# shoeffner/ann3depth

Measured on AMD Instinct MI355X. Metric: images/sec (640x480->55x74 MSDN train step), higher is better.
Workload: dtype f32

## Files before the change

### ann3depth_amd/_lib.py

```python
import collections
import ctypes
import os
from ctypes import c_char_p, c_float, c_int, c_int32, c_int64, c_size_t, c_uint8, c_uint32, c_void_p, POINTER

LIB_PATH = os.environ.get('A3D_LIB') or os.path.join(os.path.dirname(os.path.abspath(__file__)), 'liba3d.so')


class A3dError(RuntimeError):
    pass


class ConvDesc(ctypes.Structure):
    _fields_ = [(n, c_int32) for n in ('n', 'h', 'w', 'c', 'k', 'r', 's', 'stride', 'pad_t', 'pad_l', 'ho', 'wo',
                                       'ldx', 'ldy', 'precision', 'storage', 'hints')]


class SecondOutput(ctypes.Structure):
    _fields_ = [('ptr', c_void_p), ('ld', c_int32), ('step', c_int32), ('offset', c_int32), ('bf16', c_int32), ('cols', c_int32)]


class ExampleView(ctypes.Structure):
    _fields_ = [('image_height', c_int64), ('image_width', c_int64), ('image_channels', c_int64),
                ('depth_height', c_int64), ('depth_width', c_int64), ('depth_channels', c_int64),
                ('image', c_void_p), ('image_bytes', c_size_t), ('depth', c_void_p), ('depth_bytes', c_size_t)]
# ... 17 lines not shown
    'a3d_conv2d_bwd_filter_ws_bytes': (c_size_t, [_D]),
    'a3d_conv2d_bwd_filter': (c_int, [_D, _P, _P, _P, _P, _P, c_size_t, _P]),
    'a3d_conv2d_fwd_prepared_filter_bytes': (c_size_t, [_D]),
    'a3d_conv2d_fwd_prepare_filter': (c_int, [_D, _P, _P, c_size_t, _P]),
    'a3d_conv2d_bwd_filter_pooled_ws_bytes': (c_size_t, [_D]),
    'a3d_conv2d_bwd_filter_pooled': (c_int, [_D, _P, _P, c_int, _P, _P, c_int, c_int, _P, _P, _P, c_size_t, _P]),
    'a3d_conv2d_bwd_both_supported': (c_int, [_D]),
    'a3d_conv2d_bwd_both_ws_bytes': (c_size_t, [_D]),
    'a3d_conv2d_bwd_both': (c_int, [_D, _P, _P, _P, _P, _P, _P, c_int, c_int, c_int, _P, _P, c_size_t, _P]),
    'a3d_dense_fwd_ws_bytes': (c_size_t, [c_int, c_int, c_int]),
    'a3d_dense_fwd': (c_int, [c_int, c_int, c_int, _P, _P, _P, _P, c_int, _P, _P, c_size_t, _P]),
    'a3d_dense_bwd_data_ws_bytes': (c_size_t, [c_int, c_int, c_int]),
    'a3d_dense_bwd_data': (c_int, [c_int, c_int, c_int, _P, _P, _P, _P, c_int, c_float, _P, c_size_t, _P]),
    'a3d_dense_bwd_filter_ws_bytes': (c_size_t, [c_int, c_int, c_int]),
    'a3d_dense_bwd_filter': (c_int, [c_int, c_int, c_int, _P, _P, _P, _P, _P, c_size_t, _P]),
    'a3d_maxpool2x2_fwd': (c_int, [c_int, c_int, c_int, c_int, _P, _P, c_int, _P, _P]),
    'a3d_maxpool2x2_bwd': (c_int, [c_int, c_int, c_int, c_int, _P, _P, c_int, _P, c_int, _P]),
    'a3d_resize_bilinear_tf1': (c_int, [c_int, c_int, c_int, c_int, _P, c_int, c_int, _P, _P]),
    'a3d_resize_bilinear_tf1_pair': (c_int, [c_int, c_int, c_int, c_int, _P, c_int, c_int, _P, c_int, _P, c_int, c_int, _P, _P]),
    'a3d_resize_bilinear_tf1_ex': (c_int, [c_int, c_int, c_int, c_int, _P, c_int, c_int, c_int, _P, c_int, _P, c_int, c_int, c_int,
                                           _P, _P]),
    'a3d_warp_bilinear_pair': (c_int, [c_int, c_int, c_int, c_int, _P, c_int, c_int, c_int, _P, c_int, _P, c_int, c_int, c_int,
                                       _P, _P, _P]),
    'a3d_extract_patches': (c_int, [c_int, c_int, c_int, c_int, _P, c_int, c_int, _P, _P]),
    'a3d_silog_loss_fwd': (c_int, [c_int, c_int, _P, _P, _P, _P, _P]),
    'a3d_silog_loss_bwd': (c_int, [c_int, c_int, _P, _P, _P, _P, _P]),
    'a3d_dropout_keep_mask': (c_int, [c_size_t, ctypes.c_uint64, ctypes.c_uint64, c_float, _P, _P]),
    'a3d_adam_apply_tf1': (c_int, [c_size_t, _P, _P, _P, _P, c_float, c_float, c_float, c_float, c_float, c_float,
                                   c_float, _P]),
    'a3d_adam_apply_tf1_flag': (c_int, [c_size_t, _P, _P, _P, _P, c_float, c_float, c_float, c_float, c_float, c_float,
                                        c_float, _P, _P]),
    'a3d_dense_fwd_ex': (c_int, [c_int, c_int, c_int, _P, _P, _P, _P, c_int, _P, c_int, c_int, _P, c_size_t, _P]),
    'a3d_dense_bwd_data_ex': (c_int, [c_int, c_int, c_int, _P, _P, _P, _P, c_int, c_float, c_int, c_int, _P, c_size_t, _P]),
    'a3d_dense_fwd_ex2': (c_int, [c_int, c_int, c_int, _P, _P, _P, _P, c_int, c_int, c_int, _P, c_int, c_int, POINTER(SecondOutput), _P,
                                  c_size_t, _P]),
    'a3d_dense_bwd_data_ex2': (c_int, [c_int, c_int, c_int, _P, _P, _P, _P, c_int, c_float, c_int, c_int, POINTER(SecondOutput), _P,
                                       c_size_t, _P]),
    'a3d_conv2d_fwd_ex2': (c_int, [_D, _P, _P, _P, _P, c_int, POINTER(SecondOutput), _P, c_size_t, _P]),
    'a3d_silog_loss_bwd_ex': (c_int, [c_int, c_int, _P, _P, _P, _P, _P, c_int, _P]),
    'a3d_depth_metrics_ws_bytes': (c_size_t, [c_int, c_int, c_int]),
    'a3d_depth_metrics': (c_int, [c_int, c_int, c_int, _P, c_int, c_int, _P, c_int, c_float, c_float, c_float, c_float, _P, _P,
                                  c_size_t, _P]),
    'a3d_cast_bf16': (c_int, [c_size_t, _P, _P, c_int, _P]),
    'a3d_cast_rows': (c_int, [c_size_t, c_int, _P, c_int, c_int, _P, c_int, c_int, _P]),
    'a3d_pad_channels_bf16': (c_int, [c_size_t, c_int, _P, c_int, _P, _P]),
    'a3d_stream_create': (c_int, [c_int, ctypes.POINTER(ctypes.c_void_p)]),
    'a3d_stream_destroy': (c_int, [_P]),
    'a3d_maxpool2x2_fwd_bf16': (c_int, [c_int, c_int, c_int, c_int, _P, c_int, _P, c_int, _P, _P]),
    'a3d_maxpool2x2_bwd_bf16': (c_int, [c_int, c_int, c_int, c_int, _P, c_int, _P, c_int, _P, c_int, _P]),
    'a3d_copy_channel_bf16': (c_int, [c_size_t, _P, c_int, c_int, _P, c_int, c_int, _P]),
    'a3d_maxpool2x2_bwd_idx_bf16': (c_int, [c_int, c_int, c_int, c_int, _P, _P, c_int, _P, c_int, _P, c_int, _P]),
    'a3d_maxpool2x2_bwd_idx_bf16s': (c_int, [c_int, c_int, c_int, c_int, _P, _P, c_int, _P, c_int, _P, c_int, _P]),
    'a3d_dense_bwd_filter_adam_tf1': (c_int, [c_int, c_int, c_int, _P, _P, _P, _P, _P, _P, _P, _P, c_float, c_float, c_float,
                                              c_float, c_float, c_float, _P]),
    'a3d_dense_bwd_filter_adam_tf1_ex': (c_int, [c_int, c_int, c_int, _P, _P, _P, _P, _P, _P, _P, _P, c_float, c_float, c_float,
                                                 c_float, c_float, c_float, c_int, _P]),
    'a3d_superpixel_mean': (c_int, [c_int, c_int, c_int, c_int, _P, c_int, _P, _P]),
    'a3d_superpixel_hist': (c_int, [c_int, c_int, c_int, _P, c_int, _P, _P]),
    'a3d_pair_similarity': (c_int, [c_int, c_int, c_int, _P, c_int, _P, _P, _P, c_int, _P, _P, c_float, _P, _P, _P]),
    'a3d_crf_loss': (c_int, [c_int, c_int, _P, _P, _P, _P, _P, c_int, c_float, _P, _P, _P, _P]),
    'a3d_crf_map': (c_int, [c_int, c_int, _P, _P, _P, _P, c_int, _P, _P, _P]),
    'a3d_sgd_apply': (c_int, [c_size_t, _P, _P, c_float, _P]),
    'a3d_conv2d_pool_fwd': (c_int, [_D, _P, _P, _P, _P, c_int, _P, c_int, _P, c_size_t, _P]),
    'a3d_maxpool2x2_bwd_idx': (c_int, [c_int, c_int, c_int, c_int, _P, _P, c_int, _P, c_int, _P, c_int, _P]),
    'a3d_copy_channel': (c_int, [c_size_t, _P, c_int, c_int, _P, c_int, c_int, _P]),
    'a3d_comm_standin': (c_int, [_P, c_size_t, _P, c_size_t, c_int, c_float, _P]),
    'a3d_timing_enable': (c_int, [c_int]),
    'a3d_timing_collect': (c_int, [POINTER(TimingRecord), c_int]),
    'a3d_timing_select': (c_int, [POINTER(TimingRecord)]),
    'a3d_crc32c': (c_uint32, [_P, c_size_t]),
    'a3d_masked_crc32c': (c_uint32, [_P, c_size_t]),
    'a3d_tfrecord_next': (c_int, [_P, c_size_t, c_int, POINTER(c_size_t), POINTER(c_size_t), POINTER(c_size_t)]),
    'a3d_example_parse': (c_int, [_P, c_size_t, POINTER(ExampleView)]),
    'a3d_decode_raw_plus_half': (c_int, [_P, c_size_t, _P]),
    'a3d_record_decode': (c_int, [_P, c_size_t, c_int, _P, c_size_t, _P, c_size_t, POINTER(ExampleView)]),
    'a3d_record_decode_u8': (c_int, [_P, c_size_t, c_int, _P, _P, c_size_t, _P, _P, c_size_t, POINTER(ExampleView),
                                     POINTER(c_int)]),
    'a3d_records_decode': (c_int, [POINTER(c_void_p), POINTER(c_size_t), c_int, c_int, POINTER(c_int64), _P, _P, _P, _P,
                                   POINTER(c_int32), c_int, POINTER(c_int32)]),
    'a3d_h2d_gather': (c_int, [_P, _P, POINTER(c_int32), c_int, c_int, c_size_t, _P]),
    'a3d_sizeof_conv_desc': (c_size_t, []),
    'a3d_example_write': (c_int64, [_P, c_int, c_int, c_int, _P, c_int, c_int, c_int, _P, c_size_t]),
}

EXT_SIGNATURES = {
    'a3dx_resize_bilinear_tf1_valid': (c_int, [c_int, c_int, c_int, c_int, _P, c_int, c_int, c_int, _P, c_int, _P, c_int, c_int,
                                               c_int, _P, c_float, c_float, _P]),
    'a3dx_warp_bilinear_pair_valid': (c_int, [c_int, c_int, c_int, c_int, _P, c_int, c_int, c_int, _P, c_int, _P, c_int, c_int,
                                              c_int, _P, _P, c_float, c_float, _P]),
    'a3dx_silog_masked_loss_fwd': (c_int, [c_int, c_int, _P, _P, _P, _P, _P]),
    'a3dx_silog_masked_loss_bwd_ex': (c_int, [c_int, c_int, _P, _P, _P, _P, _P, c_int, _P]),
}

PAIR_SIGNATURES = {
    'a3dp_crf_loss_grad': (c_int, [c_int, c_int, _P, _P, _P, _P, _P, c_int, c_float, _P, _P, _P, _P, _P]),
    'a3dp_pair_dense_bwd': (c_int, [c_int, c_int, c_int, _P, _P, _P, _P, _P]),
    'a3dp_sgd_apply_floor': (c_int, [c_size_t, _P, _P, c_float, c_float, _P]),
}

TEXTURE_SIGNATURES = {
    'a3dt_superpixel_lbp_hist': (c_int, [c_int, c_int, c_int, _P, c_int, _P, _P]),
    'a3dt_pair_similarity3': (c_int, [c_int, c_int, c_int, _P, c_int, _P, _P, _P, _P, c_int, _P, _P, c_float, _P, _P, _P]),
}

GRADLOSS_SIGNATURES = {
    'a3dg_silog_grad_loss_fwd': (c_int, [c_int, c_int, c_int, _P, _P, c_int, c_float, _P, _P, _P]),
    'a3dg_silog_grad_loss_bwd_ex': (c_int, [c_int, c_int, c_int, _P, _P, c_int, c_float, _P, _P, _P, c_int, _P]),
}

BERHU_SIGNATURES = {
    'a3dh_berhu_loss_fwd': (c_int, [c_int, c_int, _P, _P, c_int, c_float, _P, _P, _P]),
    'a3dh_berhu_loss_bwd_ex': (c_int, [c_int, c_int, _P, _P, c_int, c_float, _P, _P, _P, c_int, _P]),
}

ALIGN_SIGNATURES = {
    'a3da_depth_align_ws_bytes': (c_size_t, [c_int, c_int, c_int, c_int]),
    'a3da_depth_align': (c_int, [c_int, c_int, c_int, _P, c_int, c_int, _P, c_int, c_float, c_float, c_int, _P, _P, _P, _P,
                                 c_size_t, _P]),
    'a3da_depth_metrics_aligned': (c_int, [c_int, c_int, c_int, _P, c_int, c_int, _P, c_int, c_float, c_float, c_float, c_float,
                                           _P, _P, _P, c_size_t, _P]),
    'a3da_affine_apply': (c_int, [c_int, c_int, _P, _P, _P, _P]),
}

SSI_SIGNATURES = {
    'a3di_ssi_loss_fwd': (c_int, [c_int, c_int, _P, _P, c_int, _P, _P, _P]),
    'a3di_ssi_loss_bwd_ex': (c_int, [c_int, c_int, _P, _P, c_int, _P, _P, _P, c_int, _P]),
}

CRF_VALID_SIGNATURES = {
    'a3dv_superpixel_mean_valid': (c_int, [c_int, c_int, c_int, _P, c_int, c_int, _P, _P, _P]),
    'a3dv_crf_loss_observed': (c_int, [c_int, c_int, _P, _P, _P, _P, _P, c_int, _P, _P, _P, _P, _P, _P, _P]),
}

FCSP_SIGNATURES = {
    'a3df_superpixel_pool_fwd': (c_int, [c_int, c_int, c_int, c_int, _P, c_int, c_int, c_int, c_int, _P, _P, _P, c_int, _P]),
    'a3df_superpixel_pool_bwd': (c_int, [c_int, c_int, c_int, c_int, _P, c_int, c_int, c_int, c_int, _P, _P, _P, c_int, _P]),
}

CRF_BAND_SIGNATURES = {
    'a3db_crf_band_nll': (c_int, [c_int, c_int, c_int, _P, _P, _P, _P, _P, c_int, _P, _P, _P, _P, _P, _P, _P]),
    'a3db_crf_band_map': (c_int, [c_int, c_int, c_int, _P, _P, _P, _P, c_int, _P, _P, _P]),
}

WINO_SIGNATURES = {
    'a3dw_conv2d_bwd_data_prepared_filter_bytes': (c_size_t, [_D]),
    'a3dw_conv2d_bwd_data_prepare_filter': (c_int, [_D, _P, _P, c_size_t, _P]),
}

WINO_GRAD_SIGNATURES = {
    'a3dwg_conv2d_bwd_filter_ws_bytes': (c_size_t, [_D]),
    'a3dwg_conv2d_bwd_filter': (c_int, [_D, _P, _P, _P, _P, _P, c_size_t, _P]),
}

class WinoBwdPool(ctypes.Structure):
    _fields_ = [('argmax', c_void_p), ('y', c_void_p), ('ldy', c_int), ('h2', c_int), ('w2', c_int)]


WINO_BWD_SIGNATURES = {
    'a3dwb_sizeof_pool': (c_size_t, []),
    'a3dwb_conv2d_bwd_ws_bytes': (c_size_t, [_D, c_int, c_int]),
    'a3dwb_conv2d_bwd': (c_int, [_D, _P, _P, _P, _P, _P, _P, _P, ctypes.POINTER(WinoBwdPool), _P, c_size_t, _P]),
}

UPSAMPLE_SIGNATURES = {
    'a3du_joint_bilateral_upsample': (c_int, [c_int, c_int, c_int, _P, c_int, c_int, _P, c_int, _P, _P, _P, _P, c_int, c_float,
                                              c_float, _P, _P]),
}

POSTERIOR_SIGNATURES = {
    'a3dc_crf_band_posterior': (c_int, [c_int, c_int, c_int, _P, _P, _P, _P, _P, c_int, _P, _P, _P, _P, _P]),
}

SLIC_SIGNATURES = {
    'a3ds_label_mean': (c_int, [c_int, c_int, c_int, c_int, _P, c_int, _P, _P, _P, _P]),
    'a3ds_label_hist': (c_int, [c_int, c_int, c_int, _P, c_int, _P, _P, _P]),
    'a3ds_slic_update': (c_int, [c_int, c_int, c_int, _P, c_int, _P, _P, _P, _P]),
    'a3ds_slic_assign': (c_int, [c_int, c_int, c_int, _P, c_int, _P, c_float, _P, _P]),
    'a3ds_slic_segment': (c_int, [c_int, c_int, c_int, _P, c_int, c_int, c_float, _P, _P, _P, _P]),
    'a3ds_pair_similarity': (c_int, [c_int, c_int, _P, _P, _P, _P, _P, c_int, _P, _P, c_float, _P, _P, _P]),
    'a3ds_label_pool_fwd': (c_int, [c_int, c_int, c_int, c_int, _P, c_int, c_int, c_int, c_int, _P, _P, _P, _P, _P, c_int, _P]),
    'a3ds_label_pool_bwd': (c_int, [c_int, c_int, c_int, c_int, _P, c_int, c_int, c_int, c_int, _P, _P, _P, _P, _P, c_int, _P]),
}

Surface = collections.namedtuple('Surface', 'prefix header signatures')
SURFACES = (
    Surface('a3d_', 'a3d.h', SIGNATURES),
    Surface('a3dx_', 'a3d_valid.h', EXT_SIGNATURES),
    Surface('a3dp_', 'a3d_pairwise.h', PAIR_SIGNATURES),
    Surface('a3dt_', 'a3d_texture.h', TEXTURE_SIGNATURES),
    Surface('a3dg_', 'a3d_gradloss.h', GRADLOSS_SIGNATURES),
    Surface('a3dv_', 'a3d_crf_valid.h', CRF_VALID_SIGNATURES),
    Surface('a3df_', 'a3d_fcsp.h', FCSP_SIGNATURES),
    Surface('a3db_', 'a3d_crf_band.h', CRF_BAND_SIGNATURES),
    Surface('a3dw_', 'a3d_wino.h', WINO_SIGNATURES),
    Surface('a3du_', 'a3d_upsample.h', UPSAMPLE_SIGNATURES),
    Surface('a3dc_', 'a3d_posterior.h', POSTERIOR_SIGNATURES),
    Surface('a3dwg_', 'a3d_wino_grad.h', WINO_GRAD_SIGNATURES),
    Surface('a3ds_', 'a3d_slic.h', SLIC_SIGNATURES),
    Surface('a3dwb_', 'a3d_wino_bwd.h', WINO_BWD_SIGNATURES),
    Surface('a3dh_', 'a3d_berhu.h', BERHU_SIGNATURES),
    Surface('a3da_', 'a3d_align.h', ALIGN_SIGNATURES),
    Surface('a3di_', 'a3d_ssi.h', SSI_SIGNATURES),
)

_lib = None


def load():
    global _lib
    if _lib is not None:
        return _lib
    if not os.path.exists(LIB_PATH):
        raise A3dError(f'{LIB_PATH} not found: build it with `python -c "import __graft_entry__ as g; g.build()"` '
                       f'or `make -C ann3depth_amd/csrc` (there is no fallback path)')
    import torch
    lib = ctypes.CDLL(LIB_PATH)
    for name, (res, args) in ((n, sig) for surface in SURFACES for n, sig in surface.signatures.items()):
        try:
            fn = getattr(lib, name)
        except AttributeError as e:
            raise A3dError(f'liba3d.so lacks symbol {name}: stale build?') from e
        fn.restype = res
        fn.argtypes = args
    if lib.a3d_sizeof_conv_desc() != ctypes.sizeof(ConvDesc):
        raise A3dError(f'liba3d.so reads a {lib.a3d_sizeof_conv_desc()}-byte a3d_conv_desc, this binding passes '
                       f'{ctypes.sizeof(ConvDesc)} bytes: stale build?')
    if lib.a3dwb_sizeof_pool() != ctypes.sizeof(WinoBwdPool):
        raise A3dError(f'liba3d.so reads a {lib.a3dwb_sizeof_pool()}-byte a3dwb_pool, this binding passes '
                       f'{ctypes.sizeof(WinoBwdPool)} bytes: stale build?')
    _lib = lib
    return lib


def last_error():
    buf = ctypes.create_string_buffer(512)
    load().a3d_last_error(buf, 512)
    return buf.value.decode(errors='replace')


def check(rc, what):
    if rc != 0:
        raise A3dError(f'{what} failed ({rc}): {last_error()}')
```

### ann3depth_amd/csrc/a3d_internal.h

```cpp
#pragma once
#include <hip/hip_runtime.h>
#include <stddef.h>
#include <stdint.h>

#include <algorithm>

#include "../../include/a3d.h"
#include "igemm_plan.h"

namespace a3d {

int set_error(int code, const char* fmt, ...);

#define A3D_CHECK_ARG(cond, ...)                                 \
  do {                                                           \
    if (!(cond)) return ::a3d::set_error(A3D_EINVAL, __VA_ARGS__); \
  } while (0)

inline void clear_stale_error() { (void)hipGetLastError(); }

inline int check_launch(const char* what) {
  hipError_t e = hipGetLastError();
  if (e != hipSuccess) return set_error(A3D_ELAUNCH, "%s: %s", what, hipGetErrorString(e));
  return A3D_OK;
}

inline unsigned grid_for(size_t total, int per_block = 256, unsigned cap = 8192) {
  size_t g = (total + per_block - 1) / per_block;
  return (unsigned)std::min<size_t>(std::max<size_t>(g, 1), cap);
}

__host__ __device__ inline bool aligned16(const void* p) { return (reinterpret_cast<uintptr_t>(p) & 15) == 0; }

struct IgemmParams;
int launch_igemm(int mode, const GemmPlan& plan, int avec, int bvec, IgemmParams& p, void* ws, hipStream_t st);
int take_second_output(IgemmParams& p, const a3d_second_output* o);

struct TimingSlot {
  hipEvent_t start, stop;
  a3d_timing_record rec;
};
bool timing_wanted(const a3d_timing_record& r);
int timing_begin(TimingSlot& slot, hipStream_t st);
void timing_end(TimingSlot& slot, hipStream_t st);
a3d_timing_record timing_record(int mode, int prec, int bm, int bn, int waves_m, int nwaves, int bk, int avec, int bvec, int lds_dma,
                                int m, int n, int k);
template <typename Launch>
int timed_launch(const a3d_timing_record& rec, hipStream_t st, Launch&& launch) {
  if (!timing_wanted(rec)) return launch();
  TimingSlot slot{};
  slot.rec = rec;
  int rc = timing_begin(slot, st);
  if (rc != A3D_OK) return rc;
  rc = launch();
  timing_end(slot, st);
  return rc;
}

bool dense_dw_applicable(int m, int k, int n);
bool dense_stream_applicable(int m, int k, int n);
size_t dense_stream_ws_bytes(int m, int k, int n);
int dense_fwd_stream(int m, int k, int n, const float* x, const float* w, const float* bias, float* y, int act,
                     const uint8_t* keep, float keep_scale, void* ws, size_t ws_bytes, hipStream_t st);
struct ReduceParams;
int launch_splitk_reduce(const ReduceParams& r, hipStream_t st);
int dense_dw_launch(int m, int k, int n, const float* x, const float* dz, float* dw, float* db, hipStream_t st);

size_t colsum_bf16_ws_bytes(int n);
bool colsum_bf16_ok(int n);
int colsum_bf16(const void* dz, int rows, int n, int ld, float* out, void* ws, int* nparts, hipStream_t st);

bool stencil1_applicable(const a3d_conv_desc* d);
size_t stencil1_bwdf_ws_bytes(const a3d_conv_desc* d);
int stencil1_fwd(const a3d_conv_desc* d, const float* x, const float* w, const float* bias, float* y, int act,
                 hipStream_t st);
int stencil1_bwd_filter(const a3d_conv_desc* d, const float* x, const float* dz, float* dw, float* db, void* ws,
                        hipStream_t st);
bool stencil1_bwd_both_applicable(const a3d_conv_desc* d);
size_t stencil1_bwd_both_ws_bytes(const a3d_conv_desc* d);
int stencil1_bwd_both(const a3d_conv_desc* d, const float* x, const float* dz, const float* w, float* dw, float* db,
                      void* dx, int lddx, int dx_bf16, int relu_mask, unsigned* state, void* ws, hipStream_t st);

bool fewch_bwdf_applicable(const a3d_conv_desc* d, bool pooled);
size_t fewch_bwdf_ws_bytes(const a3d_conv_desc* d, bool pooled);
bool fewch_extents_ok(const a3d_conv_desc* d, bool pooled, int ldz, int esz, int ld_arg);
int fewch_bwd_filter(const a3d_conv_desc* d, const float* x, int src, const void* dz, int ldz, const void* pooled_act,
                     const uint8_t* argmax, int ld_arg, float* dw, float* db, void* ws, hipStream_t st);

int fewch_reduce_launch(const float* slabs, int splits, int Mp, int NP, int M, int N, float* dw, float* db, hipStream_t st);
bool fewch16_bwdf_applicable(const a3d_conv_desc* d, bool pooled);
size_t fewch16_bwdf_ws_bytes(const a3d_conv_desc* d, bool pooled);
int fewch16_bwd_filter(const a3d_conv_desc* d, const float* x, bool pooled, const void* dz, int ldz, const void* pooled_act,
                       const uint8_t* argmax, int ld_arg, float* dw, float* db, void* ws, hipStream_t st);

bool conv3_applicable(const a3d_conv_desc* d, unsigned x_off);
size_t conv3_ws_bytes(const a3d_conv_desc* d);
int conv3_pack(const a3d_conv_desc* d, const float* w, float* wp, hipStream_t st);
int conv3_fwd(const a3d_conv_desc* d, const float* x, const float* w, const float* bias, float* y, int act, int pool,
              int ld_out, uint8_t* argmax, void* ws, size_t ws_bytes, hipStream_t st, bool prepared = false);

bool conv3b_applicable(const a3d_conv_desc* d);
size_t conv3b_filter_bytes(const a3d_conv_desc* d);
int conv3b_pack(const a3d_conv_desc* d, const float* w, void* wp, hipStream_t st);
int conv3b_fwd(const a3d_conv_desc* d, const void* x, const float* w, const float* bias, void* y, int act, int pool, int ld_out,
               uint8_t* argmax, void* ws, size_t ws_bytes, hipStream_t st, bool prepared);

struct WinoGeom {
  int oh, ow, th, tw;
  size_t T;
  int K, N, Kp, Np;
  size_t v_bytes, m_bytes, u_bytes;
};
WinoGeom wino_geom(const a3d_conv_desc* d, bool bwd);
bool wino_applicable(const a3d_conv_desc* d);
int wino_filter(const a3d_conv_desc* d, bool bwd, const float* w, float* U, hipStream_t st);
int wino_input(const a3d_conv_desc* d, bool bwd, const float* src, float* V, hipStream_t st);
int wino_output(const a3d_conv_desc* d, bool bwd, const float* M, float* out, const float* bias, const float* mask, int act,
                hipStream_t st);
a3d_timing_record wino_record(int mode, const WinoGeom& g);
int wino_gemm(IgemmParams& p, const WinoGeom& g, hipStream_t st);

struct WinoGradGeom {
  size_t T;
  int Cp, Kp;
  int splits;
  size_t v_bytes, z_bytes;
  size_t slab_bytes, bias_bytes;
};
int wino_grad_splits(int C, int K, size_t T);
WinoGradGeom wino_grad_geom(const a3d_conv_desc* d);
bool wino_grad_applicable(const a3d_conv_desc* d);
int wino_dz(const a3d_conv_desc* d, const float* dz, float* Z, hipStream_t st);
int wino_dw(const a3d_conv_desc* d, const WinoGradGeom& g, const float* slabs, const float* bparts, float* dw, float* db, hipStream_t st);
a3d_timing_record wino_grad_record(const a3d_conv_desc* d, const WinoGradGeom& g);
int wino_grad_gemm(IgemmParams& p, const WinoGradGeom& g, hipStream_t st);

struct WinoBwdPool {
  const uint8_t* argmax;
  const float* y;
  int ldy, h2, w2;
};
int wino_bwd_transforms(const a3d_conv_desc* d, const float* x, const float* dz, float* Vx, float* Vdz, float* Z, hipStream_t st);
int wino_bwd_gemm(IgemmParams& pf, const WinoGradGeom& gg, IgemmParams& pd, const WinoGeom& g, hipStream_t st);
int wino_bwd_finish(const a3d_conv_desc* d, const WinoGradGeom& gg, const float* slabs, const float* bparts, float* dw, float* db,
                    const float* M, float* dx, const float* mask, const WinoBwdPool* pool, hipStream_t st);

}
```

### ann3depth_amd/csrc/igemm.h

```cpp
#pragma once
#include <hip/hip_runtime.h>
#include <stdint.h>

#include <type_traits>

#include "igemm_plan.h"

namespace a3d {

#ifdef A3D_STAMPS
#define A3D_STAMP(var)                                                                         \
  do {                                                                                         \
    __builtin_amdgcn_sched_barrier(0);                                                         \
    unsigned long long t_;                                                                     \
    asm volatile("s_memtime %0\n\ts_waitcnt lgkmcnt(0)" : "=s"(t_)::"memory");                 \
    __builtin_amdgcn_sched_barrier(0);                                                         \
    var = t_;                                                                                  \
  } while (0)
#define A3D_RTSTAMP(var)                                                                       \
  do {                                                                                         \
    __builtin_amdgcn_sched_barrier(0);                                                         \
    unsigned long long t_;                                                                     \
    asm volatile("s_memrealtime %0\n\ts_waitcnt lgkmcnt(0)" : "=s"(t_)::"memory");             \
    __builtin_amdgcn_sched_barrier(0);                                                         \
// ... 918 lines not shown
    const int kt = kt_begin + it;
    const bool more = it + 1 < nkt;
    A3D_STAMP(s0);
    if (AHEAD) issue();
    else prepare(uni_c, std::true_type{}, kt + 1, (it + 1) % 3, more);
    __builtin_amdgcn_sched_barrier(0);
    A3D_STAMP(s1);
    if (AHEAD) prepare(uni_c, std::false_type{}, kt + 2, (it + 2) % 3, it + 2 < nkt);
    if (MODE == MODE_BWD_F) {
      if (tid < Cfg::PIX) pixtab[((it + 2) % 3) * Cfg::PIX + tid] = row_entry((kt + 2) * BK + tid, image_of((kt + 2) * BK));
    }
    const float* Ac = As + cur * Cfg::A_ELEMS;
    const float* Bc = Bs + cur * Cfg::B_ELEMS;
    if (MODE == MODE_BWD_F && do_bias) {
#pragma unroll 8
      for (int k = 0; k < BK; ++k) bsum += Bc[k * Cfg::B_LD + (tid ^ (Cfg::B_SWZ ? 32 * ((k >> 2) & 1) : 0))];
    }
    constexpr bool PIPE = (MODE != MODE_FWD) && NWAVES == 8 && BN == 128;
    if constexpr (PIPE) {
      f32x4 af[2][TM], bf[2][TN];
      auto read_frags = [&](int u, int buf) {
        const int kk = 8 * u + 4 * lh;
#pragma unroll
        for (int a = 0; a < TM; ++a) {
          const int row = (wm * Cfg::WM + a * 32 + li) ^ (Cfg::A_SWZ ? 32 * lh : 0);
          if (MODE == MODE_BWD_F) {
#pragma unroll
            for (int j = 0; j < 4; ++j) af[buf][a][j] = Ac[(kk + j) * Cfg::A_LD + row];
          } else {
            af[buf][a] = *reinterpret_cast<const f32x4*>(Ac + row * Cfg::A_LD + kk);
          }
        }
#pragma unroll
        for (int b = 0; b < TN; ++b) {
          const int col = (wn * Cfg::WN + b * 32 + li) ^ (Cfg::B_SWZ ? 32 * lh : 0);
          if (MODE == MODE_BWD_D) {
            bf[buf][b] = *reinterpret_cast<const f32x4*>(Bc + col * Cfg::B_LD + kk);
          } else {
#pragma unroll
            for (int j = 0; j < 4; ++j) bf[buf][b][j] = Bc[(kk + j) * Cfg::B_LD + col];
          }
        }
      };
      read_frags(0, 0);
#pragma unroll
      for (int u = 0; u < BK / 8; ++u) {
        constexpr int LAST = BK / 8 - 1;
        if (u < LAST) read_frags(u + 1, (u + 1) & 1);
        if (u == LAST) {
          A3D_STAMP(s2);
          if (more) store_tiles(cur ^ 1);
          A3D_STAMP(s3);
        }
#pragma unroll
        for (int j = 0; j < 4; ++j)
#pragma unroll
          for (int a = 0; a < TM; ++a)
#pragma unroll
            for (int b = 0; b < TN; ++b)
              acc[a][b] = __builtin_amdgcn_mfma_f32_32x32x2f32(af[u & 1][a][j], bf[u & 1][b][j], acc[a][b], 0, 0, 0);
        if (u < LAST) {
          constexpr int NREADS = (MODE == MODE_BWD_F ? 4 * (TM + TN) : TM + TN);
          constexpr int NMFMA = 4 * TM * TN;
          constexpr int PER = (NREADS + NMFMA - 1) / NMFMA;
#pragma unroll
          for (int i = 0; i < NMFMA; ++i) {
            __builtin_amdgcn_sched_group_barrier(0x008, 1, 0);
            __builtin_amdgcn_sched_group_barrier(0x100, PER, 0);
          }
        }
      }
    } else {
#pragma unroll
    for (int u = 0; u < BK / 8; ++u) {
      f32x4 af[TM], bf[TN];
      const int kk = 8 * u + 4 * lh;
#pragma unroll
      for (int a = 0; a < TM; ++a) {
        const int row = (wm * Cfg::WM + a * 32 + li) ^ (Cfg::A_SWZ ? 32 * lh : 0);
        if (MODE == MODE_BWD_F) {
#pragma unroll
          for (int j = 0; j < 4; ++j) af[a][j] = Ac[(kk + j) * Cfg::A_LD + row];
        } else {
          af[a] = *reinterpret_cast<const f32x4*>(Ac + row * Cfg::A_LD + kk);
        }
      }
#pragma unroll
      for (int b = 0; b < TN; ++b) {
        const int col = (wn * Cfg::WN + b * 32 + li) ^ (Cfg::B_SWZ ? 32 * lh : 0);
        if (MODE == MODE_BWD_D) {
          bf[b] = *reinterpret_cast<const f32x4*>(Bc + col * Cfg::B_LD + kk);
        } else {
#pragma unroll
          for (int j = 0; j < 4; ++j) bf[b][j] = Bc[(kk + j) * Cfg::B_LD + col];
        }
      }
      if (u == BK / 8 - 1) {
        A3D_STAMP(s2);
        if (more) store_tiles(cur ^ 1);
        A3D_STAMP(s3);
      }
#pragma unroll
      for (int j = 0; j < 4; ++j)
#pragma unroll
        for (int a = 0; a < TM; ++a)
#pragma unroll
          for (int b = 0; b < TN; ++b)
            acc[a][b] = __builtin_amdgcn_mfma_f32_32x32x2f32(af[a][j], bf[b][j], acc[a][b], 0, 0, 0);
    }
    }
    A3D_STAMP(s4);
    __syncthreads();
    A3D_STAMP(s5);
#ifdef A3D_STAMPS
    d01 += s1 - s0; d12 += s2 - s1; d23 += s3 - s2; d34 += s4 - s3; d45 += s5 - s4;
#endif
  };
  for (int it = 0; it < nkt; it += 2) {
    tile_body(it, std::integral_constant<int, 0>{});
    if (it + 1 < nkt) tile_body(it + 1, std::integral_constant<int, 1>{});
  }
  };
  if constexpr (MODE == MODE_BWD_F) {
    k_loop(std::false_type{});
  } else {
    if (p.uni) k_loop(std::true_type{});
    else k_loop(std::false_type{});
  }
#ifdef A3D_STAMPS
  A3D_STAMP(tend);
  A3D_RTSTAMP(rtend);
  if (p.stamps && lane == 0) {
    unsigned long long* o = p.stamps + ((size_t)bid_in * NWAVES + wave) * 16;
    o[0] = d01; o[1] = d12; o[2] = d23; o[3] = d34; o[4] = d45; o[5] = tend - tbeg; o[6] = (unsigned long long)nkt; o[7] = tp1 - t_entry; o[15] = tp2 - tp1;
    o[8] = tbeg - t_entry; o[9] = t_entry; o[10] = tend; o[12] = rtend - rtbeg; o[13] = rtbeg; o[14] = rtend;
  }
#define A3D_STAMP_EXIT()                                                                                   \
  do {                                                                                                     \
    unsigned long long t_exit_;                                                                            \
    A3D_STAMP(t_exit_);                                                                                    \
    if (p.stamps && lane == 0) p.stamps[((size_t)bid_in * NWAVES + wave) * 16 + 11] = t_exit_;              \
  } while (0)
#else
#define A3D_STAMP_EXIT() do { } while (0)
#endif

  igemm_epilogue<MODE, BM, BN, TM, TN, Cfg::WM, Cfg::WN>(p, acc, split, bid, seg, kt_begin, kt_end, nk_total, do_bias, bsum, tid, wave, lane,
                                                          m0, n0, wm, wn);
  }
  A3D_STAMP_EXIT();
}

template <int MODE, int BM, int BN, int WAVES_M, int NWAVES>
__global__ __launch_bounds__(256) void igemm_fixup_kernel(const IgemmParams p, const uint32_t nblk) {
  constexpr int WAVES_N = NWAVES / WAVES_M, WM = BM / WAVES_M, WN = BN / WAVES_N, TM = WM / 32, TN = WN / 32;
  constexpr int UNITS = NWAVES * TM * TN * 4;
  constexpr int MAXC = 1024;
  __shared__ uint32_t slots[MAXC];
  __shared__ uint32_t nslots;
  const int lane = threadIdx.x & 63;
  const int unit = (int)blockIdx.y * 4 + (int)(threadIdx.x >> 6);
  const uint32_t tile = blockIdx.x;
  const uint32_t nk = p.div_nk.d, tiles = (uint32_t)(p.tiles_m * p.tiles_n);
  if (threadIdx.x == 0) {
    uint32_t n = 0;
    const uint32_t total = tiles * nk, t0 = tile * nk, t1 = t0 + nk - 1;
    uint32_t jf = (uint32_t)(((unsigned long long)t0 * nblk) / total), jl = (uint32_t)(((unsigned long long)t1 * nblk) / total);
    while (jf + 1 < nblk && sk_first(jf + 1, nblk, total) <= t0) ++jf;
    while (jl + 1 < nblk && sk_first(jl + 1, nblk, total) <= t1) ++jl;
    for (uint32_t b = jf; b <= jl; ++b) {
      const uint32_t f = sk_first(b, nblk, total);
      if (f == sk_first(b + 1, nblk, total)) continue;
      if (n < MAXC) slots[n] = 2 * b + (f / nk == tile ? 0u : 1u);
      ++n;
    }
    nslots = n < MAXC ? n : MAXC;
  }
  __syncthreads();
  const uint32_t n = nslots;
  if (n <= 1) return;
  const int tile_m = (int)tile / p.tiles_n, tile_n = (int)tile - tile_m * p.tiles_n;
  if (unit < UNITS) {
    const size_t uoff = ((size_t)unit * 64 + lane) * 4;
    f32x4 s = {0.f, 0.f, 0.f, 0.f};
    auto slab_of = [&](uint32_t i) -> f32x4 {
      return *reinterpret_cast<const f32x4*>(p.sk_ws + (size_t)slots[i] * (size_t)(BM * BN) + uoff);
    };
    uint32_t i = 0;
    for (; i + 8 <= n; i += 8) {
      f32x4 v[8];
#pragma unroll
      for (int u = 0; u < 8; ++u) v[u] = slab_of(i + u);
#pragma unroll
      for (int u = 0; u < 8; ++u) s += v[u];
    }
    if (i + 4 <= n) {
      const f32x4 v0 = slab_of(i), v1 = slab_of(i + 1), v2 = slab_of(i + 2), v3 = slab_of(i + 3);
      s += v0; s += v1; s += v2; s += v3;
      i += 4;
    }
    for (; i < n; ++i) s += slab_of(i);
    const int q = unit & 3, ab = unit >> 2, bb = ab % TN, a = (ab / TN) % TM, wave = ab / (TN * TM);
    const int wm = wave / WAVES_N, wn = wave % WAVES_N, li = lane & 31, lh = lane >> 5;
    store_quad<MODE>(p, s, tile_m * BM + wm * WM + a * 32 + 8 * q + 4 * lh, tile_n * BN + wn * WN + bb * 32 + li, p.C,
                     p.ldc, false);
  }
  if (MODE == MODE_BWD_F && p.dbias != nullptr && tile_m == 0 && blockIdx.y == 0 && (int)threadIdx.x < BN) {
    static_assert(BN <= 256, "bias sums by the first 256 threads");
    float bsum = 0.f;
    for (uint32_t i = 0; i < n; ++i) bsum += p.sk_bias[(size_t)slots[i] * BN + threadIdx.x];
    if (tile_n * BN + (int)threadIdx.x < p.N) p.dbias[tile_n * BN + threadIdx.x] = bsum;
  }
}

template <int MODE, int BM, int BN, int WAVES_M, int NWAVES, int BKT, int AVEC, int BVEC>
__global__ __launch_bounds__(64 * NWAVES, (BKT == 16 ? 3 : 2) * NWAVES / 4) void igemm_kernel(const IgemmParams p) {
  igemm_body<MODE, BM, BN, WAVES_M, NWAVES, BKT, AVEC, BVEC>(p, gridDim.x, blockIdx.x);
}

struct IgemmMulti {
  IgemmParams p[4];
};
template <int MODE, int BM, int BN, int WAVES_M, int NWAVES, int BKT, int AVEC, int BVEC>
__global__ __launch_bounds__(64 * NWAVES, (BKT == 16 ? 3 : 2) * NWAVES / 4) void igemm_multi_kernel(const IgemmMulti ps) {
  const IgemmParams& p = ps.p[blockIdx.y];
  const uint32_t nwg = (uint32_t)(p.tiles_m * p.tiles_n * p.splitk);
  if (blockIdx.x >= nwg) return;
  igemm_body<MODE, BM, BN, WAVES_M, NWAVES, BKT, AVEC, BVEC>(p, nwg, blockIdx.x);
}

struct ReduceParams {
  const float* ws; float* C; const float* bias; const float* mask; const uint8_t* keep; float mask_scale;
  int M, N, ldc, splitk, act, mode, mask_act; size_t slab;
  int sub_step, sub_ph, sub_pw, outW, outHW; FastDiv div_phw, div_pw;
  int vec4;
  int c16;
  const float* dbias_ws; float* dbias_out;
  int dbias_splits;
  unsigned dbias_block0;
  void* C2; int ld2, step2, off2, c2_16, cols2;
  int c_cols;
  int row_rl, row_rlp;
};
__global__ __launch_bounds__(256) void splitk_reduce_kernel(const ReduceParams p);

}
```

### ann3depth_amd/csrc/igemm_host.hip

```cpp
#include <algorithm>
#include <cmath>

#include "../../include/a3d_wino.h"
#include "../../include/a3d_wino_grad.h"
#include "../../include/a3d_wino_bwd.h"
#include "a3d_internal.h"
#include "igemm.h"
#include "igemm_cfgs.h"

namespace a3d {

int launch_igemm_multi_bwd_d(int avec, int bvec, IgemmMulti& ps, unsigned grid_x, unsigned count, hipStream_t st);
int launch_igemm_bf16_multi_bwd_d(int bn, IgemmMulti& ps, unsigned grid_x, unsigned count, hipStream_t st);


struct RunForm {
  int vec;
  int rl, rlp;
  int kp;
  int np;
  size_t bytes;
};
static bool run_form_ok(const a3d_conv_desc* d, unsigned x_off, RunForm* rf, bool bwd_filter = false) {
  if (d->pad_t || d->pad_l || d->ldx != d->c || d->c % 4 == 0 || d->c > 4) return false;
  const int step = d->stride * d->c, row = d->w * d->c;
  int vec = 0;
  bool anywhere = false;
  if (step % 4 == 0 && row % 4 == 0 && x_off == 0) vec = 4;
  else if (step % 2 == 0 && row % 2 == 0 && (x_off & 7) == 0) vec = 2;
  else if (bwd_filter && d->precision == A3D_PREC_F32 && !d->storage && (x_off & 3) == 0) {
    vec = 2;
    anywhere = true;
  }
  if (vec == 4 && d->precision == A3D_PREC_F32) {
    const int rl = d->s * d->c;
    const int kp4 = d->r * ((rl + 3) / 4 * 4), kp2 = d->r * ((rl + 1) / 2 * 2);
    if ((kp2 + 127) / 128 < (kp4 + 127) / 128) vec = 2;
  }
  if (!vec) return false;
  rf->vec = vec;
  rf->rl = d->s * d->c;
  rf->rlp = (rf->rl + vec - 1) / vec * vec;
  rf->kp = d->r * rf->rlp;
  rf->np = (d->k + 3) / 4 * 4;
  rf->bytes = ((size_t)rf->kp * rf->np * 4 + 255) / 256 * 256;
  if (anywhere) return (d->wo - 1) * step + rf->rl <= row && (d->ho - 1) * d->stride + d->r <= d->h;
  return (d->wo - 1) * step + rf->rlp <= row;
}

__global__ __launch_bounds__(256) void pad_filter_kernel(const float* w, float* wp, int r, int rl, int rlp, int n, int np) {
  const int total = r * rlp * np;
  for (int i = blockIdx.x * 256 + threadIdx.x; i < total; i += gridDim.x * 256) {
    const int col = i % np, row = i / np;
    const int q = row % rlp, rr = row / rlp;
    wp[i] = (q < rl && col < n) ? w[(size_t)(rr * rl + q) * n + col] : 0.f;
  }
}
__global__ __launch_bounds__(256) void unpad_filter_kernel(const float* wp, float* w, int r, int rl, int rlp, int n) {
  const int total = r * rl * n;
  for (int i = blockIdx.x * 256 + threadIdx.x; i < total; i += gridDim.x * 256) {
    const int col = i % n, row = i / n;
    const int q = row % rl, rr = row / rl;
    w[i] = wp[(size_t)(rr * rlp + q) * n + col];
  }
}

struct Operands {
  bool known = false;
  unsigned x = 0, w = 0, y = 0;
  unsigned aux = 0;
  int act = A3D_ACT_NONE, pool = 0, ld_out = 0;
  bool argmax = false, prepared = false;
  bool db = true;
};
static const Operands kOnGrid{};
static Operands launch_operands(const void* x, const void* w, const void* y, const void* aux) {
  auto off16 = [](const void* p) { return (unsigned)(reinterpret_cast<uintptr_t>(p) & 15); };
  Operands o;
  o.known = true;
  o.x = off16(x); o.w = off16(w); o.y = off16(y); o.aux = off16(aux);
  return o;
}

enum GemmForm { kAsStored, kLdsDma, kRunForm, kBf16Image };
struct Route {
  bool ok = false;
  RunForm rf{};
  GemmProblem g{};
  GemmPlan plan{};
  size_t repack = 0;
  size_t bytes = 0;
};
static size_t upto(size_t need, const Route& r) { return r.ok ? std::max(need, r.bytes) : need; }
static void fit_workspace(Route& r, const Operands& o, size_t ws_bytes, size_t per_split = 0) {
  if (r.bytes <= ws_bytes || !(o.x | o.w | o.y | o.aux) || r.repack > ws_bytes) return;
  r.plan = plan_within(r.g, r.plan, ws_bytes - r.repack, per_split);
  r.bytes = r.repack + r.plan.ws_bytes + (r.plan.splitk > 1 ? (size_t)r.plan.splitk * per_split : 0);
}
#define A3D_CHECK_WS(ws, who) A3D_CHECK_ARG(aligned16(ws), who ": ws must be 16-byte aligned")

static const int kAll16 = A3D_STORE_X_BF16 | A3D_STORE_W_BF16 | A3D_STORE_Y_BF16;
static bool stored16(const a3d_conv_desc* d, int bits) { return (d->storage & bits) == bits; }
static bool ring_ok(const a3d_conv_desc* d, const Operands& o, int both, unsigned out_off, int taps) {
  if (d->precision != A3D_PREC_BF16 || !stored16(d, both) || d->c % 8 || d->k % 8) return false;
  return !o.known || (d->ldx % 8 == 0 && d->ldy % 8 == 0 && taps <= 128 && !out_off);
}

static int ilog2_exact(int v) {
  for (int l = 0; l < 8; ++l)
    if ((1 << l) == v) return l;
  return -1;
}

static int check_desc(const a3d_conv_desc* d) {
  A3D_CHECK_ARG(d != nullptr, "conv: null descriptor");
  A3D_CHECK_ARG(d->n > 0 && d->h > 0 && d->w > 0 && d->c > 0 && d->k > 0 && d->r > 0 && d->s > 0, "conv: bad dims");
  A3D_CHECK_ARG(ilog2_exact(d->stride) >= 0 && d->stride <= 4, "conv: stride %d unsupported (1, 2 or 4)", d->stride);
  A3D_CHECK_ARG(d->pad_t >= 0 && d->pad_l >= 0 && d->pad_t < d->r && d->pad_l < d->s, "conv: bad padding");
  A3D_CHECK_ARG(d->ho > 0 && d->wo > 0, "conv: bad output size");
  A3D_CHECK_ARG((d->ho - 1) * d->stride - d->pad_t < d->h && (d->wo - 1) * d->stride - d->pad_l < d->w,
                "conv: output size inconsistent with input");
  A3D_CHECK_ARG(d->ldx >= d->c && d->ldy >= d->k, "conv: pixel strides smaller than channel counts");
  A3D_CHECK_ARG(d->precision >= A3D_PREC_F32 && d->precision <= A3D_PREC_F32_WINOGRAD, "conv: unknown precision %d", d->precision);
  const double lim = 2147483647.0;
  A3D_CHECK_ARG((double)d->n * d->h * d->w * d->ldx < lim && (double)d->n * d->ho * d->wo * d->ldy < lim &&
                    (double)d->r * d->s * d->c * d->k < lim,
                "conv: tensor too large for 31-bit indexing");
  auto tile_span_ok = [&](double rows_per_image, double image_elems) {
    const double images = std::min((double)d->n, std::floor(255.0 / rows_per_image) + 2.0);
    return images * image_elems * 4.0 < lim;
  };
  A3D_CHECK_ARG(tile_span_ok((double)d->ho * d->wo, (double)d->h * d->w * d->ldx) &&
                    tile_span_ok(std::max(1.0, std::floor((double)d->h / d->stride) * std::floor((double)d->w / d->stride)),
                                 (double)d->ho * d->wo * d->ldy),
                "conv: single images too large for 31-bit byte offsets inside a tile");
  return A3D_OK;
}

#define A3D_AS_F32(d)                                          \
  a3d_conv_desc d##_f32;                                       \
  if ((d) && (d)->precision == A3D_PREC_F32_WINOGRAD) {        \
    d##_f32 = *(d);                                            \
    d##_f32.precision = A3D_PREC_F32;                          \
    (d) = &d##_f32;                                            \
  }

static GemmProblem fwd_problem(const a3d_conv_desc* d) {
  GemmProblem g;
  g.mode = MODE_FWD;
  g.M = d->n * d->ho * d->wo; g.N = d->k; g.K = d->r * d->s * d->c;
  g.avec = (d->c % 4 == 0 && d->ldx % 4 == 0) ? 4 : 1;
  g.bvec = (d->k % 4 == 0) ? 4 : 1;
  return g;
}
static GemmProblem bwd_d_problem(const a3d_conv_desc* d) {
  GemmProblem g;
  g.mode = MODE_BWD_D;
  g.M = d->n * d->h * d->w; g.N = d->c; g.K = d->r * d->s * d->k;
// ... 648 lines not shown
  fill_common(p, r.g);
  rc = apply_storage(p, d->precision, d->storage & A3D_STORE_X_BF16, d->storage & A3D_STORE_Y_BF16, false, d->c, d->ldx, -1, d->ldy,
                     x, dz, dw, "x", "dz", "dw");
  if (rc != A3D_OK) return rc;
  A3D_CHECK_ARG(!d->storage || plan.prec == A3D_PREC_BF16, "conv2d_bwd_filter: bf16 storage needs vectorisable operands");
  if (r.bytes > ws_bytes) return set_error(A3D_EWORKSPACE, "conv2d_bwd_filter: need %zu workspace bytes", r.bytes);
  hipStream_t st = static_cast<hipStream_t>(stream);
  if (plan.ring && db) {
    float* parts = reinterpret_cast<float*>(static_cast<char*>(ws) + plan.ws_bytes);
    int nparts = 0;
    rc = colsum_bf16(dz, r.g.K, d->k, d->ldy, plan.splitk > 1 ? nullptr : db, parts, &nparts, st);
    if (rc != A3D_OK) return rc;
    if (plan.splitk > 1) { p.dbias_parts = parts; p.dbias_parts_out = db; p.dbias_parts_n = nparts; }
    db = nullptr;
  }
  p.A = x; p.B = dz; p.C = out; p.dbias = db;
  p.npix = r.g.K; p.nrsc = r.g.M;
  fill_gather(p, d, d->ldx, run ? 1 : d->s, run ? rf.rlp : d->c);
  p.ldb = d->ldy; p.ldc = d->k;
  fill_staging(p, MODE_BWD_F, (unsigned long long)d->n * d->h * d->w * d->ldx, (unsigned long long)d->n * d->ho * d->wo * d->ldy, d->r,
               run ? 1 : d->s);
  if (run) { p.unpad_dst = dw; p.unpad_rl = rf.rl; p.unpad_rlp = rf.rlp; }
  rc = launch_igemm(MODE_BWD_F, plan, r.g.avec, r.g.bvec, p, static_cast<char*>(ws) + r.repack, st);
  if (rc != A3D_OK || !run || p.unpad_done) return rc;
  clear_stale_error();
  hipLaunchKernelGGL(unpad_filter_kernel, dim3((d->r * rf.rl * d->k + 255) / 256), dim3(256), 0, st, out, dw, d->r,
                     rf.rl, rf.rlp, d->k);
  return check_launch("unpad_filter");
}

static bool wino_grad_takes(const a3d_conv_desc* d) { return check_desc(d) == A3D_OK && wino_grad_applicable(d); }

static IgemmParams wino_grad_product(const WinoGradGeom& g, const float* V, const float* Z, float* slabs, float* bparts) {
  a3d_conv_desc e{};
  e.n = (int)g.T; e.h = e.w = e.ho = e.wo = 1; e.c = g.Cp; e.k = g.Kp; e.r = e.s = 1; e.stride = 1; e.ldx = g.Cp; e.ldy = g.Kp;
  GemmProblem gp = bwd_f_problem(&e);
  IgemmParams p;
  fill_common(p, gp);
  p.A = V; p.B = Z; p.C = slabs; p.dbias = bparts;
  p.npix = gp.K; p.nrsc = gp.M;
  fill_gather(p, &e, g.Cp, 1, g.Cp);
  p.ldb = g.Kp; p.ldc = g.Kp;
  fill_staging(p, MODE_BWD_F, (unsigned long long)g.T * g.Cp, (unsigned long long)g.T * g.Kp, 1, 1);
  return p;
}

size_t a3dwg_conv2d_bwd_filter_ws_bytes(const a3d_conv_desc* d) {
  if (!wino_grad_takes(d)) return a3d_conv2d_bwd_filter_ws_bytes(d);
  const WinoGradGeom g = wino_grad_geom(d);
  return g.v_bytes + g.z_bytes + g.slab_bytes + g.bias_bytes;
}

int a3dwg_conv2d_bwd_filter(const a3d_conv_desc* d, const float* x, const float* dz, float* dw, float* db, void* ws,
                            size_t ws_bytes, void* stream) {
  if (!wino_grad_takes(d)) return a3d_conv2d_bwd_filter(d, x, dz, dw, db, ws, ws_bytes, stream);
  A3D_CHECK_ARG(x && dz && dw, "conv2d_bwd_filter (Winograd): null tensor");
  A3D_CHECK_WS(ws, "conv2d_bwd_filter (Winograd)");
  const WinoGradGeom g = wino_grad_geom(d);
  const size_t need = g.v_bytes + g.z_bytes + g.slab_bytes + g.bias_bytes;
  if (!ws || need > ws_bytes) return set_error(A3D_EWORKSPACE, "conv2d_bwd_filter (Winograd): need %zu workspace bytes", need);
  hipStream_t st = static_cast<hipStream_t>(stream);
  char* base = static_cast<char*>(ws);
  float* V = reinterpret_cast<float*>(base);
  float* Z = reinterpret_cast<float*>(base + g.v_bytes);
  float* slabs = reinterpret_cast<float*>(base + g.v_bytes + g.z_bytes);
  float* bparts = reinterpret_cast<float*>(base + g.v_bytes + g.z_bytes + g.slab_bytes);
  int rc = wino_input(d, false, x, V, st);
  if (rc != A3D_OK) return rc;
  rc = wino_dz(d, dz, Z, st);
  if (rc != A3D_OK) return rc;
  IgemmParams p = wino_grad_product(g, V, Z, slabs, db ? bparts : nullptr);
  rc = timed_launch(wino_grad_record(d, g), st, [&] { return wino_grad_gemm(p, g, st); });
  if (rc != A3D_OK) return rc;
  return wino_dw(d, g, slabs, bparts, dw, db, st);
}

static bool wino_bwd_takes(const a3d_conv_desc* d) {
  if (!wino_grad_takes(d)) return false;
  const WinoGeom gx = wino_geom(d, false), gd = wino_geom(d, true);
  return gx.th <= gd.th && gx.tw <= gd.tw;
}
static a3d_conv_desc as_winograd(const a3d_conv_desc* d) {
  a3d_conv_desc e = *d;
  e.precision = A3D_PREC_F32_WINOGRAD;
  return e;
}

size_t a3dwb_sizeof_pool(void) { return sizeof(a3dwb_pool); }

size_t a3dwb_conv2d_bwd_ws_bytes(const a3d_conv_desc* d, int w_prepared, int pooled) {
  (void)pooled;
  if (!wino_bwd_takes(d)) return std::max(a3dwg_conv2d_bwd_filter_ws_bytes(d), a3d_conv2d_bwd_data_ws_bytes(d));
  const a3d_conv_desc e = as_winograd(d);
  const WinoGradGeom g = wino_grad_geom(&e);
  return wino_bytes(&e, true, w_prepared != 0) + g.v_bytes + g.z_bytes + g.slab_bytes + g.bias_bytes;
}

int a3dwb_conv2d_bwd(const a3d_conv_desc* d, const float* x, const float* dz, const float* w_or_U, float* dw, float* db, float* dx,
                     const float* relu_mask, const a3dwb_pool* pool, void* ws, size_t ws_bytes, void* stream) {
  static_assert(sizeof(WinoBwdPool) == sizeof(a3dwb_pool), "WinoBwdPool mirrors a3dwb_pool");
  if (!wino_bwd_takes(d)) {
    A3D_CHECK_ARG(!pool, "conv2d_bwd (Winograd): a pool only where the Winograd routes take the descriptor");
    const int rc = a3dwg_conv2d_bwd_filter(d, x, dz, dw, db, ws, ws_bytes, stream);
    return rc != A3D_OK ? rc : a3d_conv2d_bwd_data(d, dz, w_or_U, dx, relu_mask, ws, ws_bytes, stream);
  }
  A3D_CHECK_ARG(x && dz && w_or_U && dw && dx, "conv2d_bwd (Winograd): null tensor");
  A3D_CHECK_WS(ws, "conv2d_bwd (Winograd)");
  A3D_CHECK_ARG(!(pool && relu_mask), "conv2d_bwd (Winograd): relu_mask and pool exclude each other");
  A3D_CHECK_ARG(!pool || (pool->argmax && pool->y && pool->ldy >= d->c && pool->h2 >= 2 && pool->w2 >= 2 && pool->h2 / 2 == d->h &&
                          pool->w2 / 2 == d->w),
                "conv2d_bwd (Winograd): the pool's halved extents must be the layer's input's");
  const a3d_conv_desc e = as_winograd(d);
  const bool prepared = (d->hints & A3D_HINT_W_PREPARED) != 0;
  const WinoGeom g = wino_geom(&e, true);
  const WinoGradGeom gg = wino_grad_geom(&e);
  const size_t need = wino_bytes(&e, true, prepared) + gg.v_bytes + gg.z_bytes + gg.slab_bytes + gg.bias_bytes;
  if (!ws || need > ws_bytes) return set_error(A3D_EWORKSPACE, "conv2d_bwd (Winograd): need %zu workspace bytes", need);
  A3D_CHECK_ARG(!prepared || aligned16(w_or_U), "conv2d_bwd (Winograd): the prepared filter must be 16-byte aligned");
  hipStream_t st = static_cast<hipStream_t>(stream);
  char* base = static_cast<char*>(ws);
  const float* U = w_or_U;
  int rc;
  if (!prepared) {
    rc = wino_filter(&e, true, w_or_U, reinterpret_cast<float*>(base), st);
    if (rc != A3D_OK) return rc;
    U = reinterpret_cast<const float*>(base);
    base += g.u_bytes;
  }
  auto take = [&base](size_t bytes) {
    float* p = reinterpret_cast<float*>(base);
    base += bytes;
    return p;
  };
  float *Vdz = take(g.v_bytes), *M = take(g.m_bytes);
  float *Vx = take(gg.v_bytes), *Z = take(gg.z_bytes), *slabs = take(gg.slab_bytes), *bparts = take(gg.bias_bytes);
  rc = wino_bwd_transforms(&e, x, dz, Vx, Vdz, Z, st);
  if (rc != A3D_OK) return rc;
  IgemmParams pf = wino_grad_product(gg, Vx, Z, slabs, db ? bparts : nullptr);
  IgemmParams pd = wino_product(g, Vdz, U, M);
  const a3d_timing_record rf = wino_grad_record(&e, gg), rd = wino_record(MODE_BWD_D, g);
  if (timing_wanted(rf) || timing_wanted(rd) || tune_int("A3D_WINO_BWD_PAIR", 1) == 0) {
    rc = timed_launch(rf, st, [&] { return wino_grad_gemm(pf, gg, st); });
    if (rc != A3D_OK) return rc;
    rc = timed_launch(rd, st, [&] { return wino_gemm(pd, g, st); });
  } else {
    rc = wino_bwd_gemm(pf, gg, pd, g, st);
  }
  if (rc != A3D_OK) return rc;
  WinoBwdPool wp{};
  if (pool) wp = WinoBwdPool{pool->argmax, pool->y, pool->ldy, pool->h2, pool->w2};
  return wino_bwd_finish(&e, gg, slabs, bparts, dw, db, M, dx, relu_mask, pool ? &wp : nullptr, st);
}

static a3d_conv_desc dense_desc(int m, int k, int n) {
  a3d_conv_desc d{};
  d.n = m; d.h = 1; d.w = 1; d.c = k; d.k = n; d.r = 1; d.s = 1; d.stride = 1; d.ho = 1; d.wo = 1;
  d.ldx = k; d.ldy = n;
  return d;
}

size_t a3d_dense_fwd_ws_bytes(int m, int k, int n) {
  a3d_conv_desc d = dense_desc(m, k, n);
  if (check_desc(&d) != A3D_OK) return 0;
  return std::max(plan_gemm(fwd_problem(&d), A3D_PREC_F32).ws_bytes, dense_stream_ws_bytes(m, k, n));
}

int a3d_dense_fwd(int m, int k, int n, const float* x, const float* w, const float* bias, float* y, int act,
                  const uint8_t* drop_keep, void* ws, size_t ws_bytes, void* stream) {
  return a3d_dense_fwd_ex(m, k, n, x, w, bias, y, act, drop_keep, A3D_PREC_F32, 0, ws, ws_bytes, stream);
}

int a3d_dense_fwd_ex(int m, int k, int n, const float* x, const float* w, const float* bias, float* y, int act,
                     const uint8_t* drop_keep, int precision, int storage, void* ws, size_t ws_bytes, void* stream) {
  return a3d_dense_fwd_ex2(m, k, n, x, w, bias, y, n, n, act, drop_keep, precision, storage, nullptr, ws, ws_bytes, stream);
}

int a3d_dense_fwd_ex2(int m, int k, int n, const float* x, const float* w, const float* bias, float* y, int ldy, int ncols_y, int act,
                      const uint8_t* drop_keep, int precision, int storage, const a3d_second_output* out2, void* ws,
                      size_t ws_bytes, void* stream) {
  A3D_CHECK_ARG(m > 0 && k > 0 && n > 0, "dense_fwd: bad dims");
  A3D_CHECK_ARG(ncols_y > 0 && ncols_y <= n && ldy >= ncols_y, "dense_fwd: y rows of %d columns at pitch %d from a GEMM of %d", ncols_y, ldy, n);
  A3D_CHECK_ARG((storage & ~(A3D_STORE_W_BF16 | A3D_STORE_X_BF16)) == 0, "dense_fwd: the weights and x may be bf16, y is float32");
  if (precision == A3D_PREC_F32_WINOGRAD) precision = A3D_PREC_F32;
  a3d_conv_desc d = dense_desc(m, k, n);
  d.precision = precision;
  int rc = check_desc(&d);
  if (rc != A3D_OK) return rc;
  A3D_CHECK_ARG(x && w && y, "dense_fwd: null tensor");
  A3D_CHECK_WS(ws, "dense_fwd");
  if (precision == A3D_PREC_F32 && !storage && dense_stream_applicable(m, k, n) && aligned16(x) && !out2 && ldy == n && ncols_y == n &&
      !tune_int("A3D_NO_DENSE_KERNELS", 0))
    return dense_fwd_stream(m, k, n, x, w, bias, y, act, drop_keep, 2.f, ws, ws_bytes, static_cast<hipStream_t>(stream));
  GemmProblem g = fwd_problem(&d);
  if (!aligned16(x)) g.avec = 1;
  if (!aligned16(w)) g.bvec = 1;
  IgemmParams p;
  fill_common(p, g);
  rc = apply_storage(p, precision, storage & A3D_STORE_X_BF16, storage & A3D_STORE_W_BF16, false, k, k, n, n, x, w, y, "x", "w", "y");
  if (rc != A3D_OK) return rc;
  A3D_CHECK_ARG(!p.a16 || aligned16(y), "dense_fwd: beside a bf16 x, y must be 16-byte aligned (the LDS-DMA kernel alone reads a bf16 x)");
  storage_vecs(g, p.a16, p.b16, p.c16);
  g.ring_ok = p.a16 && p.b16 && precision == A3D_PREC_BF16 && k % 8 == 0 && n % 8 == 0 && aligned16(y) && act != A3D_ACT_SIGMOID;
  g.need_reduce = ncols_y != n;
  GemmPlan plan = plan_gemm(g, precision);
  if (!aligned16(x) || !aligned16(w) || !aligned16(y)) plan = plan_within(g, plan, ws ? ws_bytes : 0, 0);
  A3D_CHECK_ARG(!storage || plan.prec == A3D_PREC_BF16, "dense_fwd: bf16 weights need vectorisable operands");
  A3D_CHECK_ARG(!p.a16 || plan.ring, "dense_fwd: a bf16 x is taken by the LDS-DMA kernel only (bf16 weights, k and n multiples of 8)");
  if (plan.ws_bytes > ws_bytes) return set_error(A3D_EWORKSPACE, "dense_fwd: need %zu workspace bytes", plan.ws_bytes);
  p.A = x; p.B = w; p.C = y; p.bias = bias; p.act = act; p.keep = drop_keep; p.mask_scale = 2.f;
  p.npix = m; p.nrsc = k;
  fill_gather(p, &d, k, 1, k);
  p.ldb = n; p.ldc = ldy; p.c_cols = ncols_y == n ? 0 : ncols_y;
  rc = take_second_output(p, out2);
  if (rc != A3D_OK) return rc;
  fill_staging(p, MODE_FWD, (unsigned long long)m * k, (unsigned long long)k * n, 1, 1);
  return launch_igemm(MODE_FWD, plan, g.avec, g.bvec, p, ws, static_cast<hipStream_t>(stream));
}

size_t a3d_dense_bwd_data_ws_bytes(int m, int k, int n) {
  a3d_conv_desc d = dense_desc(m, k, n);
  return a3d_conv2d_bwd_data_ws_bytes(&d);
}

int a3d_dense_bwd_data(int m, int k, int n, const float* dz, const float* w, float* dx, const float* mask,
                       int mask_act, float scale, void* ws, size_t ws_bytes, void* stream) {
  return a3d_dense_bwd_data_ex(m, k, n, dz, w, dx, mask, mask_act, scale, A3D_PREC_F32, 0, ws, ws_bytes, stream);
}

int a3d_dense_bwd_data_ex(int m, int k, int n, const float* dz, const float* w, float* dx, const float* mask, int mask_act,
                          float scale, int precision, int storage, void* ws, size_t ws_bytes, void* stream) {
  return a3d_dense_bwd_data_ex2(m, k, n, dz, w, dx, mask, mask_act, scale, precision, storage, nullptr, ws, ws_bytes, stream);
}

int a3d_dense_bwd_data_ex2(int m, int k, int n, const float* dz, const float* w, float* dx, const float* mask, int mask_act,
                           float scale, int precision, int storage, const a3d_second_output* out2, void* ws, size_t ws_bytes,
                           void* stream) {
  A3D_CHECK_ARG(m > 0 && k > 0 && n > 0, "dense_bwd_data: bad dims");
  if (precision == A3D_PREC_F32_WINOGRAD) precision = A3D_PREC_F32;
  A3D_CHECK_ARG(precision >= A3D_PREC_F32 && precision <= A3D_PREC_BF16, "dense_bwd_data: unknown precision %d", precision);
  A3D_CHECK_ARG(!mask || mask_act == A3D_ACT_RELU || mask_act == A3D_ACT_SIGMOID, "dense_bwd_data: bad mask_act");
  a3d_conv_desc d = dense_desc(m, k, n);
  int rc = check_desc(&d);
  if (rc != A3D_OK) return rc;
  A3D_CHECK_ARG(dz && w && dx, "dense_bwd_data: null tensor");
  A3D_CHECK_WS(ws, "dense_bwd_data");
  GemmProblem g = bwd_d_problem(&d);
  if (!aligned16(dz)) g.avec = 1;
  if (!aligned16(w)) g.bvec = 1;
  IgemmParams p;
  fill_common(p, g);
  rc = apply_storage(p, precision, storage & A3D_STORE_Y_BF16, storage & A3D_STORE_W_BF16, storage & A3D_STORE_X_BF16, n, n, n, n, dz, w,
                     dx, "dz", "w", "dx");
  if (rc != A3D_OK) return rc;
  A3D_CHECK_ARG(!p.c16 || aligned16(mask), "dense_bwd_data: bf16 mask must be 16-byte aligned");
  storage_vecs(g, p.a16, p.b16, p.c16);
  g.ring_ok = p.a16 && p.b16 && precision == A3D_PREC_BF16 && k % 8 == 0 && n % 8 == 0 && aligned16(dx) &&
              (!mask || (aligned16(mask) && mask_act == A3D_ACT_RELU));
  GemmPlan plan = plan_gemm(g, precision);
  if (!aligned16(dz) || !aligned16(w) || !aligned16(dx) || !aligned16(mask)) plan = plan_within(g, plan, ws ? ws_bytes : 0, 0);
  A3D_CHECK_ARG(!storage || plan.prec == A3D_PREC_BF16, "dense_bwd_data: bf16 weights need vectorisable operands");
  A3D_CHECK_ARG(!(p.a16 || p.c16) || plan.ring, "dense_bwd_data: bf16 dz / dx are taken by the LDS-DMA kernel only (bf16 weights, k and n multiples of 8, ReLU mask)");
  if (plan.ws_bytes > ws_bytes) return set_error(A3D_EWORKSPACE, "dense_bwd_data: need %zu workspace bytes", plan.ws_bytes);
  p.A = dz; p.B = w; p.C = dx; p.mask = mask; p.mask_scale = scale; p.mask_act = mask_act;
  p.npix = m; p.nrsc = n;
  fill_gather(p, &d, n, 1, n);
  p.Cn = k;
  p.ldc = k;
  p.S_full = 1;
  rc = take_second_output(p, out2);
  if (rc != A3D_OK) return rc;
  fill_staging(p, MODE_BWD_D, (unsigned long long)m * n, (unsigned long long)k * n, 1, 1);
  return launch_igemm(MODE_BWD_D, plan, g.avec, g.bvec, p, ws, static_cast<hipStream_t>(stream));
}

size_t a3d_dense_bwd_filter_ws_bytes(int m, int k, int n) {
  a3d_conv_desc d = dense_desc(m, k, n);
  return a3d_conv2d_bwd_filter_ws_bytes(&d);
}

int a3d_dense_bwd_filter(int m, int k, int n, const float* x, const float* dz, float* dw, float* db, void* ws,
                         size_t ws_bytes, void* stream) {
  A3D_CHECK_ARG(m > 0 && k > 0 && n > 0, "dense_bwd_filter: bad dims");
  A3D_CHECK_WS(ws, "dense_bwd_filter");
  if (dense_dw_applicable(m, k, n) && (long)k * n >= (1L << 16) && !tune_int("A3D_NO_DENSE_KERNELS", 0)) {
    A3D_CHECK_ARG(x && dz && dw, "dense_bwd_filter: null tensor");
    return dense_dw_launch(m, k, n, x, dz, dw, db, static_cast<hipStream_t>(stream));
  }
  a3d_conv_desc d = dense_desc(m, k, n);
  return a3d_conv2d_bwd_filter(&d, x, dz, dw, db, ws, ws_bytes, stream);
}

}
```

### ann3depth_amd/models.py

```python
import collections
import contextlib
import ctypes
import math
import os

import numpy as np
import torch

from . import _lib, augment as augment_, ops
from ._lib import ConvDesc
from .feed import DeviceFeed

NET_H, NET_W = 228, 304
OUT_H, OUT_W = 55, 74
SAMPLES_COARSE = 2000000
SAMPLES_FINE = 1500000

ConvSpec = collections.namedtuple('ConvSpec', 'name cin cout k stride padding relu')

MSDN_CONVS = [
    ConvSpec('coarse/conv/conv2d_0', 3, 96, 11, 4, 'VALID', True),
    ConvSpec('coarse/conv/conv2d_1', 96, 256, 5, 1, 'SAME', True),
    ConvSpec('coarse/conv/conv2d_2', 256, 384, 3, 1, 'SAME', True),
    ConvSpec('coarse/conv/conv2d_3', 384, 384, 3, 1, 'SAME', True),
# ... 134 lines not shown
    objective = 'silog'

    def __init__(self, batchsize, device='cuda', params=None, seed=3000, global_step=0, beta2=1.0, reducer=None,
                 precision='fp32', keep_dense_grads=True, overlap=True, valid_range=None, grad_weight=0.0,
                 objective='silog', berhu_fraction=0.2):
        if objective not in MSDN_OBJECTIVES:
            raise ValueError(f"objective {objective!r}: {', '.join(map(repr, MSDN_OBJECTIVES[:-1]))} or {MSDN_OBJECTIVES[-1]!r}")
        berhu_fraction = float(berhu_fraction)
        if not 0 < berhu_fraction <= 1:
            raise ValueError(f'berhu_fraction {berhu_fraction!r}: the threshold is a fraction in (0, 1] of the largest error')
        grad_weight = float(grad_weight)
        if not grad_weight >= 0:
            raise ValueError(f'grad_weight {grad_weight!r}: the weight of the gradient-matching term is a number >= 0')
        if objective != 'silog' and grad_weight > 0:
            raise ValueError(f"objective {objective!r} with grad_weight {grad_weight!r}: the gradient-matching term is defined "
                             f'on log differences and belongs to the silog objective')
        self.grad_weight = grad_weight
        self.valid_range = check_valid_range(valid_range)
        self._loss = msdn_loss_launches(objective, berhu_fraction, grad_weight, self.valid_range is not None)
        vars(self).update(self._loss.attrs)
        self.keep_dense_grads = keep_dense_grads or reducer is not None or batchsize > 64
        self.bf16s = precision == 'bf16s'
        self._c4_32_fresh = False
        if self.bf16s:
            precision = 'bf16'
        self.precision = precision
        self.B = B = batchsize
        self.device = torch.device(device)
        self.global_step = global_step
        self.reducer = reducer
        dev = self.device
        self.overlap = overlap
        self._shared_desc = {}
        self._prep = {}
        self._alone = ()
        self._deferred = None
        self._m_sharded = False
        self.dense_exchange = None
        if reducer is not None:
            want = os.environ.get('A3D_DP_DENSE', 'scatter')
            if want not in ('scatter', 'allreduce'):
                raise ValueError(f'A3D_DP_DENSE={want!r}: scatter or allreduce')
            self.dense_exchange = 'reduce_scatter' if (want == 'scatter' and reducer.inplace_ok(dev)) else 'all_reduce'
            if want == 'scatter' and self.dense_exchange == 'all_reduce':
                print('MSDNReplica: in-place reduce-scatter failed its self-check on this backend; the dense bucket is '
                      'all-reduced instead', flush=True)
        self._dense_pieces = None
        self._poison = None
        self._poison_seen = []
        self.fuse_pool = precision == 'fp32'
        self.side = None
        if self.overlap and dev.type == 'cuda':
            handle = ctypes.c_void_p()
            with torch.cuda.device(dev):
                ops.check(_lib.load().a3d_stream_create(1, ctypes.byref(handle)), 'a3d_stream_create')
            self.side = torch.cuda.ExternalStream(handle.value, device=dev)
            self._side_handle = handle.value
        shapes = collections.OrderedDict()
        for c in MSDN_CONVS:
            shapes[c.name + '/kernel'] = (c.k, c.k, c.cin, c.cout)
            shapes[c.name + '/bias'] = (c.cout,)
        for n, i, o in MSDN_DENSES:
            shapes[n + '/kernel'] = (i, o)
            shapes[n + '/bias'] = (o,)
        self.shapes = shapes
        self.groups = collections.OrderedDict()
        self.group_of = {}
        for gname, (lr, scopes) in MSDN_OPTIMIZERS.items():
            gshapes = collections.OrderedDict((n, s) for n, s in shapes.items()
                                              if any(n.startswith(sc + '/') for sc in scopes))
            world = reducer.world_size if (reducer is not None and gname == 'CoarseDense') else 1
            self.groups[gname] = ParamGroup(gname, lr, gshapes, dev, beta2=beta2, multiple=world)
            for n in gshapes:
                self.group_of[n] = gname
        if params is None:
            rng = np.random.default_rng(seed)
            params = {n: (glorot_uniform(rng, s) if n.endswith('/kernel') else np.zeros(s, np.float32))
                      for n, s in shapes.items()}
        self.load_params(params)

        def buf(*shape):
            return torch.empty(shape, device=dev)

        def abuf(*shape):
            return torch.empty(shape, device=dev, dtype=torch.bfloat16 if self.bf16s else torch.float32)
        self.conv = {c.name: c for c in MSDN_CONVS}
        self.x = buf(B, NET_H, NET_W, 3)
        self.t = buf(B, OUT_H, OUT_W, 1)
        self.c0 = None if self.bf16s else buf(B, 55, 74, 96)
        self.c1 = None if self.bf16s else buf(B, 27, 37, 256)
        self.p0 = abuf(B, 27, 37, 96); self.p1 = abuf(B, 13, 18, 256)
        self.c2 = abuf(B, 13, 18, 384); self.c3 = abuf(B, 13, 18, 384); self.c4 = abuf(B, 6, 8, 256)
        self.drop = buf(B, 4096)
        self.coarse = buf(B, OUT_H, OUT_W, 1)
        self.f1 = buf(B, 110, 148, 63) if not self.bf16s else None
        self.cat = abuf(B, OUT_H, OUT_W, 64)
        self.f2 = buf(B, OUT_H, OUT_W, 64)
        self.fine = buf(B, OUT_H, OUT_W, 1)
        width, name = self._loss.width, self._loss.name
        self.loss_out_c = buf(width); self.loss_out_f = buf(width)
        self.loss_coarse = self.loss_out_c[:1]; self.loss_fine = self.loss_out_f[:1]
        if width >= 2:
            self.loss_pair_c = self.loss_out_c[:2]; self.loss_pair_f = self.loss_out_f[:2]
        if width == 4:
            setattr(self, f'loss_{name}_c', self.loss_out_c); setattr(self, f'loss_{name}_f', self.loss_out_f)
        self.a0 = torch.empty((B, 27, 37, 96), dtype=torch.uint8, device=dev)
        self.a1 = torch.empty((B, 13, 18, 256), dtype=torch.uint8, device=dev)
        self.af1 = torch.empty((B, OUT_H, OUT_W, 63), dtype=torch.uint8, device=dev)
        self.pooled_fwd = None
        self.ws_c = self._loss.ws(B, dev); self.ws_f = self._loss.ws(B, dev)
        self.t_one = buf(B, 1, 1, 1) if valid_range is not None else None
        self.dz1 = buf(B, OUT_H * OUT_W); self.dz0 = buf(B, 4096)
        self.dc4 = abuf(B, 6, 8, 256); self.dc3 = abuf(B, 13, 18, 384); self.dc2 = abuf(B, 13, 18, 384)
        self.dp1 = abuf(B, 13, 18, 256); self.dc1 = abuf(B, 27, 37, 256)
        self.dp0 = abuf(B, 27, 37, 96); self.dc0 = None
        self.dfine = buf(B, OUT_H, OUT_W, 1); self.df2 = abuf(B, OUT_H, OUT_W, 64)
        self.dcat = abuf(B, OUT_H, OUT_W, 64); self.df1 = None
        if self.bf16s:
            self.c4_32 = buf(B, 6, 8, 256)
            self.dz0_16 = torch.empty((B, 4096), device=dev, dtype=torch.bfloat16)
            self.dense_bf16_x = B <= 64
            if not self.dense_bf16_x:
                self.dc4_32 = buf(B, 6, 8, 256)
            NP = (OUT_H * OUT_W + 7) // 8 * 8
            self.w1pad = torch.zeros((4096, NP), device=dev, dtype=torch.bfloat16)
            self.b1pad = torch.zeros((1, NP), device=dev)
            self.drop16 = torch.empty((B, 4096), device=dev, dtype=torch.bfloat16)
            self.dz1_16 = torch.zeros((B, NP), device=dev, dtype=torch.bfloat16)
        def D(*a):
            return ops.conv_desc(*a, precision=precision)
        self.d = {
            'coarse/conv/conv2d_0': D(B, NET_H, NET_W, 3, 96, 11, 11, 4, 'VALID'),
            'coarse/conv/conv2d_1': D(B, 27, 37, 96, 256, 5, 5, 1, 'SAME'),
            'coarse/conv/conv2d_2': D(B, 13, 18, 256, 384, 3, 3, 1, 'SAME'),
            'coarse/conv/conv2d_3': D(B, 13, 18, 384, 384, 3, 3, 1, 'SAME'),
            'coarse/conv/conv2d_4': D(B, 13, 18, 384, 256, 3, 3, 2, 'VALID'),
            'fine/first/conv2d': D(B, NET_H, NET_W, 3, 63, 9, 9, 2, 'VALID'),
            'fine/second/conv2d': D(B, OUT_H, OUT_W, 64, 64, 5, 5, 1, 'SAME'),
            'fine/third': D(B, OUT_H, OUT_W, 64, 1, 5, 5, 1, 'SAME'),
        }
        self.d_wino = {}
        if precision == 'fp32' and dev.type == 'cuda':
            for n in self.WINO_LAYERS:
                d = self.d[n]
                if d.n * -(-d.ho // 2) * -(-d.wo // 2) >= self.WINO_MIN_TILES:
                    e = self.d_wino[n] = ConvDesc.from_buffer_copy(d)
                    e.precision = ops.PREC['fp32w']
        self.wino_grad = set()
        if precision == 'fp32' and dev.type == 'cuda':
            for n in self.WINO_GRAD_LAYERS:
                d = self.d[n]
                if d.n * -(-d.ho // 2) * -(-d.wo // 2) >= self.WINO_GRAD_MIN_TILES:
                    self.wino_grad.add(n)
        self.d_few = {}
        if dev.type == 'cuda':
            few_prec = 'bf16' if self.bf16s else 'fp32'
            for n, dd in (('coarse/conv/conv2d_0', ops.conv_desc(B, NET_H, NET_W, 3, 96, 11, 11, 4, 'VALID', precision=few_prec)),
                          ('fine/first/conv2d', ops.conv_desc(B, NET_H, NET_W, 3, 63, 9, 9, 2, 'VALID', precision=few_prec))):
                if ops.conv2d_bwd_filter_pooled_supported(dd):
                    self.d_few[n] = dd
        self.store = {}
        self.wcopy = {}
        if self.bf16s:
            X, W, Y = ops.STORE_X, ops.STORE_W, ops.STORE_Y
            for n in ('coarse/conv/conv2d_1', 'coarse/conv/conv2d_2', 'coarse/conv/conv2d_3', 'coarse/conv/conv2d_4'):
                self.store[n] = {'fwd': X | W | Y, 'bwd_d': X | W | Y, 'bwd_f': X | Y}
            self.store['coarse/conv/conv2d_0'] = {'bwd_f': Y}
            self.d['fine/first/conv2d'].precision = ops.PREC['fp32']
            self.store['fine/second/conv2d'] = {'fwd': X | W, 'bwd_d': W | X | Y, 'bwd_f': X | Y}
            self.x4 = torch.empty((B, NET_H, NET_W, 4), device=dev, dtype=torch.bfloat16)
            self.w0_4 = torch.zeros((11, 11, 4, 96), device=dev)
            self.d0_4 = ops.with_storage(ops.conv_desc(B, NET_H, NET_W, 4, 96, 11, 11, 4, 'VALID', ldy=96, precision='bf16'),
                                         X | Y)
            self.w4 = torch.zeros((9, 9, 4, 63), device=dev)
            self.d4 = ops.with_storage(ops.conv_desc(B, NET_H, NET_W, 4, 63, 9, 9, 2, 'VALID', ldy=64, precision='bf16'),
                                       X | Y)
            for n in list(self.store) + ['coarse/dense/dense_0']:
                if n == 'coarse/dense/dense_0' or self.store[n].get('fwd', 0) & W:
                    self.wcopy[n] = torch.empty(self.shapes[n + '/kernel'], device=dev, dtype=torch.bfloat16)
            self.refresh_weight_copies()

    def __del__(self):
        handle, self._side_handle = getattr(self, '_side_handle', None), None
        if handle:
            try:
                torch.cuda.synchronize(self.device)
                ops.drop_workspace(handle)
                _lib.load().a3d_stream_destroy(handle)
            except Exception:
                pass

    SHARE_CU = ('fine/first/conv2d', 'fine/second/conv2d')
    WINO_LAYERS = ('coarse/conv/conv2d_2', 'coarse/conv/conv2d_3')
    WINO_MIN_TILES = 504
    WINO_GRAD_LAYERS = WINO_LAYERS
    WINO_GRAD_MIN_TILES = 504
    WINO_BWD_CHAIN = True

    def _desc(self, name, which):
        d = self.d[name]
        bits = self.store.get(name, {}).get(which, 0)
        if which == 'fwd' and self.side is not None and name in self.SHARE_CU and name not in self._alone:
            key = (name, bits)
            if key not in self._shared_desc:
                e = ops.with_storage(d, bits)
                e.hints = ops.HINT_SHARE_CU
                self._shared_desc[key] = e
            return self._shared_desc[key]
        return ops.with_storage(d, bits) if bits else d

    def _w(self, name, which='fwd'):
        if name in self.wcopy and (name not in self.store or self.store[name][which] & ops.STORE_W):
            return self.wcopy[name]
        return self._v(name + '/kernel')

    def _prepared(self, key, desc, w, which='fwd'):
        if self.device.type != 'cuda':
            return desc, w
        pf = self._prep.get(key)
        if pf is None:
            pf = self._prep[key] = ops.PreparedFilter(desc, self.device, which)
            pf.source = w
            if pf.ok:
                pf.refresh(w)
        return (pf.desc_prepared, pf.buf) if pf.ok else (desc, w)

    def _refresh_prepared(self):
        for pf in self._prep.values():
            if pf.ok:
                pf.refresh(pf.source)

    def refresh_weight_copies(self):
        for n, c in self.wcopy.items():
            ops.cast_bf16(self._v(n + '/kernel'), c)
        if self.bf16s:
            self.w4[:, :, :3, :] = self._v('fine/first/conv2d/kernel')
            self.w0_4[:, :, :3, :] = self._v('coarse/conv/conv2d_0/kernel')
            n = 'coarse/dense/dense_1'
            ops.cast_rows(self._v(n + '/kernel'), self.w1pad)
            ops.cast_rows(self._v(n + '/bias').view(1, -1), self.b1pad)

    def _weights_moved(self, *groups):
        if not all(g.frozen() for g in groups):
            if self.wcopy:
                self.refresh_weight_copies()
            self._refresh_prepared()

    def settle(self):
        if self._deferred is not None:
            works, group, scale = self._deferred
            self._deferred = None
            if works and isinstance(works[0], tuple):
                self._poll_poison()
                for work, a, b in works:
                    self.reducer.wait(work)
                    group.apply_slice(a, b, scale, poisoned=self._poison)
                group.advance()
                self._m_sharded = True
                self._watch_poison()
                return
            for work in works:
                self.reducer.wait(work)
            group.apply(scale)
            self._weights_moved(group)

    def _dense_buckets(self):
        if self._dense_pieces is None:
            gd = self.groups['CoarseDense']
            q = self.reducer.world_size * ParamGroup.ALIGN
            c = -(-gd.offsets['coarse/dense/dense_1/kernel'][0] // q) * q
            third = -(-(c // 3) // q) * q
            self._dense_pieces = ([(c, gd.count)], [(0, third), (third, 2 * third), (2 * third, c)])
        return self._dense_pieces

    def _my_slice(self, a, b):
        n = (b - a) // self.reducer.world_size
        return a + self.reducer.rank * n, a + (self.reducer.rank + 1) * n

    def _watch_poison(self):
        red = self.reducer
        work = red.any(self._poison)
        red.wait(work)
        if not hasattr(self, '_poison_ring'):
            ring = torch.empty(4, dtype=torch.int32)
            self._poison_ring = (ring.pin_memory() if self.device.type == 'cuda' else ring, 0)
        ring, nxt = self._poison_ring
        self._poison_ring = (ring, (nxt + 1) % 4)
        host = ring[nxt:nxt + 1]
        host.copy_(self._poison, non_blocking=True)
        ev = None
        if self.device.type == 'cuda':
            ev = torch.cuda.Event()
            ev.record()
        self._poison_seen.append((ev, host))

    def _poll_poison(self, block=False):
        while self._poison_seen and (block or len(self._poison_seen) >= 2):
            ev, host = self._poison_seen.pop(0)
            if ev is not None:
                ev.synchronize()
            if int(host.item()):
                self._resync()

    def _resync(self):
        gd = self.groups['CoarseDense']
        early, late = self._dense_buckets()
        for a, b in early + late:
            for buf in (gd.var, gd.v, gd.m):
                self.reducer.all_gather(buf[a:b])
        self._poison.zero_()
        self._poison_seen = []
        self._m_sharded = False

    def gather_state(self):
        self.settle()
        if self._m_sharded:
            self._poll_poison(block=True)
        if self._m_sharded:
            gd = self.groups['CoarseDense']
            early, late = self._dense_buckets()
            for a, b in early + late:
                self.reducer.all_gather(gd.m[a:b])
            self._m_sharded = False

    def load_params(self, params):
        self.settle()
        for n, shp in self.shapes.items():
            g = self.groups[self.group_of[n]]
            a = np.asarray(params[n], np.float32)
            assert a.shape == tuple(shp), (n, a.shape, shp)
            g.view(g.var, n).copy_(torch.from_numpy(np.ascontiguousarray(a)))
        if getattr(self, 'wcopy', None):
            self.refresh_weight_copies()
        if getattr(self, '_prep', None):
            self._refresh_prepared()

    def _v(self, name):
        g = self.groups[self.group_of[name]]
        return g.view(g.var, name)

    def _g(self, name):
        g = self.groups[self.group_of[name]]
        return g.view(g.grad, name)

    def var(self, name):
        self.settle()
        return self._v(name)

    def grad(self, name):
        self.settle()
        return self._g(name)
# ... 115 lines not shown
        if self.side is not None:
            torch.cuda.current_stream().wait_stream(self.side)

    def prepool_equivalent(self, which):
        src = {'c0': (self.c0, self.p0, self.a0, 1), 'c1': (self.c1, self.p1, self.a1, 1),
               'f1': (self.f1, self.cat, self.af1, 2)}[which]
        full, pooled, arg, phase = src
        if self.pooled_fwd != phase and not self.bf16s:
            return full
        if full is None:
            full = torch.empty((pooled.shape[0],) + {'c0': (55, 74, 96), 'c1': (27, 37, 256), 'f1': (110, 148, 63)}[which],
                               device=self.device)
        pooled = pooled.float()
        c = arg.shape[-1]
        out = torch.zeros_like(full)
        ph, pw = arg.shape[1], arg.shape[2]
        win = out[:, :2 * ph, :2 * pw, :].reshape(full.shape[0], ph, 2, pw, 2, c)
        a = arg.long()
        for pos in range(4):
            win[:, :, pos >> 1, :, pos & 1, :] = torch.where(a == pos, pooled[..., :c], torch.zeros_like(pooled[..., :c]))
        return out

    def _conv_pool(self, name, x, y_pooled, argmax=None):
        d, w = self._fwd_operands(name)
        ops.conv2d_pool_fwd(d, x, w, self._v(name + '/bias'), y_pooled, 'relu', argmax)

    def _fine_first_image_form(self, argmax=None):
        d, w = self._prepared(('fine/first/image', 0, 0, 0), self.d4, self.w4)
        ops.conv2d_pool_fwd(d, self.x4, w, self._v('fine/first/conv2d/bias'), self.cat, 'relu', argmax)

    def forward(self, images, depths, keep_mask, join=True, phase=None, warp=None):
        if depths is None:
            pass
        elif self.valid_range is not None:
            lo, hi = self.valid_range
            if warp is not None:
                ops.warp_bilinear_pair_valid(images, self.x, depths, self.t, warp, lo, hi)
            elif images.shape[:3] == depths.shape[:3]:
                ops.resize_bilinear_tf1_pair_valid(images, self.x, depths, self.t, lo, hi)
            else:
                ops.resize_bilinear_tf1(images, self.x)
                ops.resize_bilinear_tf1_valid(depths, self.t, lo, hi, scratch=self.t_one)
        elif warp is not None:
            ops.warp_bilinear_pair(images, self.x, depths, self.t, warp)
        elif images.shape[:3] == depths.shape[:3]:
            ops.resize_bilinear_tf1_pair(images, self.x, depths, self.t)
        else:
            ops.resize_bilinear_tf1(images, self.x)
            ops.resize_bilinear_tf1(depths, self.t)
        B = self.B
        self.dropout_on = keep_mask is not None
        self._alone = ('fine/second/conv2d',) if phase == 2 else ()
        if self.bf16s:
            ops.pad_channels_bf16(self.x, self.x4)
        fused = self.fuse_pool and phase in (1, 2, 3)
        self.pooled_fwd = phase if fused else None
        lean_fine = fused
        if fused:
            train = phase == 1
            self._conv_pool('coarse/conv/conv2d_0', self.x, self.p0, self.a0 if train else None)
            self._conv_pool('coarse/conv/conv2d_1', self.p0, self.p1, self.a1 if train else None)
        elif self.bf16s:
            d, w = self._prepared(('conv2d_0/image', 0, 0, 0), self.d0_4, self.w0_4)
            ops.conv2d_pool_fwd(d, self.x4, w, self._v('coarse/conv/conv2d_0/bias'), self.p0, 'relu', self.a0)
            self._conv_pool('coarse/conv/conv2d_1', self.p0, self.p1, self.a1)
        else:
            self._conv('coarse/conv/conv2d_0', self.x, self.c0)
            ops.maxpool2x2_fwd(self.c0, self.p0)
            self._conv('coarse/conv/conv2d_1', self.p0, self.c1)
            ops.maxpool2x2_fwd(self.c1, self.p1)
        def fine_first():
            with self._beside():
                if lean_fine:
                    self._conv_pool('fine/first/conv2d', self.x, self.cat, self.af1 if phase == 2 else None)
                elif self.bf16s:
                    self._fine_first_image_form(None if phase in (1, 3) else self.af1)
                else:
                    self._conv('fine/first/conv2d', self.x, self.f1)
        self._conv('coarse/conv/conv2d_2', self.p1, self.c2)
        self._conv('coarse/conv/conv2d_3', self.c2, self.c3)
        fine_first()
        self._c4_32_fresh = False
        if self.bf16s and self.dense_bf16_x and phase == 1:
            n4 = 'coarse/conv/conv2d_4'
            ops.conv2d_fwd(self._desc(n4, 'fwd'), self.c3, self._w(n4), self._v(n4 + '/bias'), self.c4, 'relu',
                           out2=ops.second_output(self.c4_32.view(-1, 256)))
            self._c4_32_fresh = True
        else:
            self._conv('coarse/conv/conv2d_4', self.c3, self.c4)
        if not self._sharded_in_flight():
            self.settle()
        w, b = self._kb('coarse/dense/dense_0')
        if self.bf16s and self.dense_bf16_x:
            ops.dense_fwd_ex(self.c4.view(B, -1), self.wcopy['coarse/dense/dense_0'], b, self.drop, 'relu',
                             drop_keep=keep_mask, precision='bf16', storage=ops.STORE_W | ops.STORE_X,
                             out2=ops.second_output(self.drop16))
        elif self.bf16s:
            ops.cast_bf16(self.c4, self.c4_32)
            ops.dense_fwd_ex(self.c4_32.view(B, -1), self.wcopy['coarse/dense/dense_0'], b, self.drop, 'relu',
                             drop_keep=keep_mask, precision='bf16', storage=ops.STORE_W)
        else:
            ops.dense_fwd(self.c4.view(B, -1), w, b, self.drop, 'relu', drop_keep=keep_mask)
        w, b = self._kb('coarse/dense/dense_1')
        cat_done = self.bf16s and self.dense_bf16_x
        if cat_done:
            ops.dense_fwd_ex(self.drop16, self.w1pad, self.b1pad, self.coarse.view(B, -1), None, precision='bf16',
                             storage=ops.STORE_W | ops.STORE_X, n=self.w1pad.shape[1],
                             out2=ops.second_output(self.cat, cols=OUT_H * OUT_W, step=64, offset=63, ld=OUT_H * OUT_W))
        else:
            ops.dense_fwd(self.drop, w, b, self.coarse.view(B, -1))
        with self._beside():
            if cat_done:
                pass
            elif lean_fine or self.bf16s:
                ops.copy_channel(self.coarse, 0, self.cat, 63)
            else:
                ops.maxpool2x2_fwd(self.f1, self.cat, extra=self.coarse)
            self._conv('fine/second/conv2d', self.cat, self.f2)
            self._conv('fine/third', self.f2, self.fine)
            if depths is not None:
                self._loss_fwd(self.fine, self.loss_out_f, self.ws_f)
        if depths is not None:
            self._loss_fwd(self.coarse, self.loss_out_c, self.ws_c)
        if join:
            self._join()

    def predict(self, images, n=None):
        B = self.B
        n = images.shape[0] if n is None else int(n)
        check_rows('predict', n, B, f'a batch of {images.shape[0]} images', images.shape[0])
        ops.resize_bilinear_tf1(images[:n], self.x[:n])
        if n < B:
            self.x[n:].zero_()
        self.forward(images, None, None, join=True, phase=3)
        return self.coarse.view(B, OUT_H, OUT_W), self.fine.view(B, OUT_H, OUT_W)

    def _loss_fwd(self, out, loss, ws):
        self._loss.fwd(out, self.t, loss, ws)

    def _loss_bwd(self, out, ws, dout, dout16=None):
        self._loss.bwd(out, self.t, ws, dout, dout16)

    def _sharded_in_flight(self):
        d = self._deferred
        return d is not None and bool(d[0]) and isinstance(d[0][0], tuple)

    def _fused_dense_adam(self):
        return not self.keep_dense_grads and self.groups['CoarseDense'].frozen()

    def _bwd_data(self, name, dz, dx, relu_mask=None):
        d, w = self._desc(name, 'bwd_d'), self._w(name, 'bwd_d')
        if name in self.d_wino:
            d, w = self._prepared((name, 'bwd_d', 'fp32w'), self.d_wino[name], w, 'bwd_d')
        ops.conv2d_bwd_data(d, dz, w, dx, relu_mask=relu_mask)

    def _wino_chain(self, name):
        return self.WINO_BWD_CHAIN and name in self.d_wino and name in self.wino_grad

    def _bwd_wino(self, name, x, dz, dx, relu_mask=None, pool=None):
        d, w = self._prepared((name, 'bwd_d', 'fp32w'), self.d_wino[name], self._w(name, 'bwd_d'), 'bwd_d')
        ops.conv2d_bwd_wino(d, x, dz, w, self._g(name + '/kernel'), self._g(name + '/bias'), dx, relu_mask=relu_mask, pool=pool)

    def _bwd_filter(self, name, x, dz):
        if name in self.d:
            call = ops.conv2d_bwd_filter_wino if name in self.wino_grad else ops.conv2d_bwd_filter
            call(self._desc(name, 'bwd_f'), x, dz, self._g(name + '/kernel'), self._g(name + '/bias'))
        elif self._fused_dense_adam():
            g = self.groups[self.group_of[name + '/kernel']]
            kw = [g.view(buf, name + '/kernel') for buf in (g.var, g.m, g.v)]
            kb = [g.view(buf, name + '/bias') for buf in (g.var, g.m, g.v)]
            ops.dense_bwd_filter_adam_tf1(x, dz, *kw, *kb, g.lr, g.beta1, g.beta2, float(g.beta1_power),
                                          float(g.beta2_power), 1.0, precision='bf16' if self.bf16s else 'fp32')
        else:
            ops.dense_bwd_filter(x, dz, self._g(name + '/kernel'), self._g(name + '/bias'))

    def backward_coarse(self, after_dense=None, after_conv2=None, after_dense1=None):
        B = self.B
        bf16_x = self.bf16s and self.dense_bf16_x
        self._loss_bwd(self.coarse, self.ws_c, self.dz1.view(B, OUT_H, OUT_W, 1),
                       dout16=self.dz1_16 if bf16_x else None)
        self.settle()
        n = 'coarse/dense/dense_1'
        self._bwd_filter(n, self.drop, self.dz1)
        if after_dense1 is not None:
            after_dense1()
        if bf16_x:
            ops.dense_bwd_data_ex(self.dz1_16, self.w1pad, self.dz0, mask=self.drop, scale=2.0 if self.dropout_on else 1.0,
                                  precision='bf16', storage=ops.STORE_W | ops.STORE_Y,
                                  out2=ops.second_output(self.dz0_16))
        else:
            ops.dense_bwd_data(self.dz1, self._v(n + '/kernel'), self.dz0, mask=self.drop, scale=2.0 if self.dropout_on else 1.0)
        n = 'coarse/dense/dense_0'
        if bf16_x and not self._c4_32_fresh:
            ops.cast_bf16(self.c4, self.c4_32)
        flat = (self.c4_32 if self.bf16s else self.c4).view(B, -1)
        self._bwd_filter(n, flat, self.dz0)
        if bf16_x:
            ops.dense_bwd_data_ex(self.dz0_16, self.wcopy[n], self.dc4.view(B, -1), mask=self.c4.view(B, -1), scale=1.0,
                                  precision='bf16', storage=ops.STORE_W | ops.STORE_X | ops.STORE_Y)
        elif self.bf16s:
            ops.dense_bwd_data_ex(self.dz0, self.wcopy[n], self.dc4_32.view(B, -1), mask=flat, scale=1.0, precision='bf16',
                                  storage=ops.STORE_W)
            ops.cast_bf16(self.dc4_32, self.dc4)
        else:
            ops.dense_bwd_data(self.dz0, self._v(n + '/kernel'), self.dc4.view(B, -1), mask=flat, scale=1.0)
        if after_dense is not None:
            after_dense()
        n = 'coarse/conv/conv2d_4'
        self._bwd_filter(n, self.c3, self.dc4)
        self._bwd_data(n, self.dc4, self.dc3, relu_mask=self.c3)
        self._join()
        dw = self._bwd_filter
        pooled = self.pooled_fwd == 1 or self.bf16s
        n = 'coarse/conv/conv2d_3'
        if self._wino_chain(n):
            self._bwd_wino(n, self.c2, self.dc3, self.dc2, relu_mask=self.c2)
        else:
            dw(n, self.c2, self.dc3)
            self._bwd_data(n, self.dc3, self.dc2, relu_mask=self.c2)
        n = 'coarse/conv/conv2d_2'
        if self._wino_chain(n):
            self._bwd_wino(n, self.p1, self.dc2, self.dc1 if pooled else self.dp1, pool=(self.a1, self.p1) if pooled else None)
            if after_conv2 is not None:
                after_conv2()
            if not pooled:
                ops.maxpool2x2_bwd(self.c1, self.dp1, self.dc1, relu_mask=True)
        else:
            dw(n, self.p1, self.dc2)
            if after_conv2 is not None:
                after_conv2()
            self._bwd_data(n, self.dc2, self.dp1)
            if pooled:
                ops.maxpool2x2_bwd_idx(self.a1, self.p1, self.dp1, self.dc1, relu_mask=True)
            else:
                ops.maxpool2x2_bwd(self.c1, self.dp1, self.dc1, relu_mask=True)
        n = 'coarse/conv/conv2d_1'
        dw(n, self.p0, self.dc1)
        self._bwd_data(n, self.dc1, self.dp0)
        n = 'coarse/conv/conv2d_0'
        if pooled and n in self.d_few:
            ops.conv2d_bwd_filter_pooled(self.d_few[n], self.x, self.dp0, self.p0, self.a0, self._g(n + '/kernel'),
                                         self._g(n + '/bias'))
            return
        if self.dc0 is None:
            self.dc0 = torch.empty((self.B, 55, 74, 96), device=self.device, dtype=self.dp0.dtype)
        if pooled:
            ops.maxpool2x2_bwd_idx(self.a0, self.p0, self.dp0, self.dc0, relu_mask=True)
        else:
            ops.maxpool2x2_bwd(self.c0, self.dp0, self.dc0, relu_mask=True)
        dw(n, self.x, self.dc0)

    def backward_fine(self):
        self._join()
        self._loss_bwd(self.fine, self.ws_f, self.dfine)
        n = 'fine/third'
        if ops.conv2d_bwd_both_supported(self.d[n]):
            ops.conv2d_bwd_both(self.d[n], self.f2, self.dfine, self._v(n + '/kernel'), self._g(n + '/kernel'),
                                self._g(n + '/bias'), self.df2, relu_mask=True)
        else:
            assert not self.bf16s, 'bf16 storage: df2 is a bf16 tensor only the fused backward writes'
            self._bwd_filter(n, self.f2, self.dfine)
            self._bwd_data(n, self.dfine, self.df2, relu_mask=self.f2)
        n = 'fine/second/conv2d'
        self._bwd_filter(n, self.cat, self.df2)
        self._bwd_data(n, self.df2, self.dcat)
        n = 'fine/first/conv2d'
        if (self.pooled_fwd == 2 or self.bf16s) and n in self.d_few:
            ops.conv2d_bwd_filter_pooled(self.d_few[n], self.x, self.dcat, self.cat, self.af1, self._g(n + '/kernel'),
                                         self._g(n + '/bias'))
            return
        if self.df1 is None:
            self.df1 = torch.empty((self.B, 110, 148, 63), device=self.device)
        if self.pooled_fwd == 2 or self.bf16s:
            ops.maxpool2x2_bwd_idx(self.af1, self.cat, self.dcat, self.df1, relu_mask=True)
        else:
            ops.maxpool2x2_bwd(self.f1, self.dcat, self.df1, relu_mask=True)
        self._bwd_filter(n, self.x, self.df1)

    def step(self, images, depths, keep_mask, warp=None):
        if keep_mask is not None and keep_mask.dtype != torch.uint8:
            keep_mask = keep_mask.to(torch.uint8)
        phase = phase_of(self.global_step, self.B)
        self.forward(images, depths, keep_mask, join=False, phase=phase, warp=warp)
        red = self.reducer
        scale = 1.0 / red.world_size if red is not None else 1.0
        if phase == 1:
            gc, gd = self.groups['CoarseConv'], self.groups['CoarseDense']
            if red is None:
                fused = self._fused_dense_adam()
                self.backward_coarse()
                gc.apply(scale)
                if fused:
                    gd.advance()
                else:
                    gd.apply(scale)
                self._weights_moved(gc, gd)
            else:
                handle, tail = [], []
                cut = gc.offsets['coarse/conv/conv2d_2/kernel'][0]
                if gd.frozen() and self.dense_exchange == 'reduce_scatter':
                    early, late = self._dense_buckets()
                    if self._poison is None:
                        self._poison = torch.zeros(1, dtype=torch.int32, device=self.device)

                    def scatter(pieces):
                        for a, b in pieces:
                            work, _ = red.reduce_scatter(gd.grad[a:b])
                            handle.append((work,) + self._my_slice(a, b))
                    after_dense1, after_dense = (lambda: scatter(early)), (lambda: scatter(late))
                else:
                    d1 = gd.offsets['coarse/dense/dense_1/kernel'][0]
                    third = -(-(d1 // 3) // ParamGroup.ALIGN) * ParamGroup.ALIGN
                    pieces0 = [(0, third), (third, 2 * third), (2 * third, d1)]
                    after_dense1 = lambda: handle.append(red.start(gd.grad[d1:]))
                    after_dense = lambda: handle.extend(red.start(gd.grad[a:b]) for a, b in pieces0)
                self.backward_coarse(after_dense1=after_dense1, after_dense=after_dense,
                                     after_conv2=lambda: tail.append(red.start(gc.grad[cut:], urgent=True)))
                head = red.start(gc.grad[:cut], urgent=True)
# ... 794 lines not shown
```

### ann3depth_amd/ops.py

```python
import collections
import ctypes

import torch

from . import _lib
from ._lib import ConvDesc, check

ACT = {None: 0, 'relu': 1, 'sigmoid': 2}
PREC = {'fp32': 0, 'f32': 0, 'bf16x3': 1, 'bf16': 2, 'fp32w': 3}


def _ptr(t):
    return None if t is None else ctypes.c_void_p(t.data_ptr())


def _stream():
    return ctypes.c_void_p(torch.cuda.current_stream().cuda_stream)


class Workspace:

    def __init__(self):
        self.buf = None

    def reserve(self, nbytes, device):
        if self.buf is None or self.buf.numel() < nbytes or self.buf.device != device:
            if torch.cuda.is_current_stream_capturing():
                raise RuntimeError(f'workspace of {nbytes} bytes must be reserved before graph capture')
            self.buf = torch.empty(max(nbytes, 1 << 20), dtype=torch.uint8, device=device)
        return self.buf

    def get(self, nbytes, device):
        buf = self.reserve(nbytes, device)
        return ctypes.c_void_p(buf.data_ptr()), buf.numel()


_WS = {}


def _ws():
    key = torch.cuda.current_stream().cuda_stream
    w = _WS.get(key)
    if w is None:
        w = _WS[key] = Workspace()
    return w


def drop_workspace(stream_handle):
    _WS.pop(stream_handle, None)


def same_pad(in_size, k, stride):
    out = -(-in_size // stride)
    pad = max((out - 1) * stride + k - in_size, 0)
    return out, pad // 2


STORE_X, STORE_W, STORE_Y = 1, 2, 4


HINT_SHARE_CU = 1
HINT_W_PREPARED = 2


class PreparedFilter:

    def __init__(self, desc, device, which='fwd'):
        lib = _lib.load()
        self.stem = {'fwd': 'a3d_conv2d_fwd', 'bwd_d': 'a3dw_conv2d_bwd_data'}[which]
        nbytes = getattr(lib, self.stem + '_prepared_filter_bytes')(ctypes.byref(desc))
        self.ok = nbytes > 0
        self.desc = desc
        if self.ok:
            self.buf = torch.empty(nbytes, dtype=torch.uint8, device=device)
            self.desc_prepared = ConvDesc.from_buffer_copy(desc)
            self.desc_prepared.hints = desc.hints | HINT_W_PREPARED

    def refresh(self, w):
        name = self.stem + '_prepare_filter'
        check(getattr(_lib.load(), name)(ctypes.byref(self.desc), _ptr(w), _ptr(self.buf), self.buf.numel(), _stream()), name)


def conv_desc(n, h, w, c, k, r, s, stride, padding, ldx=None, ldy=None, precision='fp32', storage=0, hints=0):
    padding = padding.upper()
    if padding == 'SAME':
        ho, pt = same_pad(h, r, stride)
        wo, pl = same_pad(w, s, stride)
    elif padding == 'VALID':
        ho, pt = (h - r) // stride + 1, 0
        wo, pl = (w - s) // stride + 1, 0
    else:
        raise ValueError(padding)
    return ConvDesc(n=n, h=h, w=w, c=c, k=k, r=r, s=s, stride=stride, pad_t=pt, pad_l=pl, ho=ho, wo=wo,
                    ldx=ldx or c, ldy=ldy or k, precision=PREC[precision], storage=storage, hints=hints)


def second_output(t, cols=None, step=1, offset=0, ld=None):
    if t is None:
        return None
    ld = t.shape[-1] if ld is None else ld
    o = _lib.SecondOutput(t.data_ptr(), ld, step, offset, int(t.dtype == torch.bfloat16), ld if cols is None else cols)
    o._keep = t
    return o


def _o2(out2):
    return None if out2 is None else ctypes.byref(out2)


def conv2d_fwd(d, x, w, bias, y, act=None, out2=None):
    lib = _lib.load()
    ws, n = _ws().get(lib.a3d_conv2d_fwd_ws_bytes(ctypes.byref(d)), x.device)
    if out2 is not None:
        check(lib.a3d_conv2d_fwd_ex2(ctypes.byref(d), _ptr(x), _ptr(w), _ptr(bias), _ptr(y), ACT[act], _o2(out2), ws, n, _stream()),
              'a3d_conv2d_fwd_ex2')
        return y
    check(lib.a3d_conv2d_fwd(ctypes.byref(d), _ptr(x), _ptr(w), _ptr(bias), _ptr(y), ACT[act], ws, n, _stream()),
          'a3d_conv2d_fwd')
    return y


def conv2d_pool_fwd(d, x, w, bias, y_pooled, act='relu', argmax=None):
    lib = _lib.load()
    ws, n = _ws().get(lib.a3d_conv2d_fwd_ws_bytes(ctypes.byref(d)), x.device)
    check(lib.a3d_conv2d_pool_fwd(ctypes.byref(d), _ptr(x), _ptr(w), _ptr(bias), _ptr(y_pooled), y_pooled.shape[-1],
                                  _ptr(argmax), ACT[act], ws, n, _stream()), 'a3d_conv2d_pool_fwd')
    return y_pooled


def maxpool2x2_bwd_idx(argmax, y_pooled, dy, dx, relu_mask=True):
    n, h, w, c = dx.shape
    if y_pooled.dtype == torch.bfloat16 and dx.dtype == torch.bfloat16:
        assert dy.dtype == torch.bfloat16
        name = 'a3d_maxpool2x2_bwd_idx_bf16s'
    elif y_pooled.dtype == torch.bfloat16:
        assert dy.dtype == torch.bfloat16 and dx.dtype == torch.float32
        name = 'a3d_maxpool2x2_bwd_idx_bf16'
    else:
        name = 'a3d_maxpool2x2_bwd_idx'
    check(getattr(_lib.load(), name)(n, h, w, c, _ptr(argmax), _ptr(y_pooled), y_pooled.shape[-1], _ptr(dy), dy.shape[-1],
                                     _ptr(dx), int(relu_mask), _stream()), name)
    return dx


def copy_channel(src, c_src, dst, c_dst):
    npix = src.numel() // src.shape[-1]
    assert dst.numel() // dst.shape[-1] == npix
    fn = _lib.load().a3d_copy_channel_bf16 if dst.dtype == torch.bfloat16 else _lib.load().a3d_copy_channel
    check(fn(npix, _ptr(src), src.shape[-1], c_src, _ptr(dst), dst.shape[-1], c_dst, _stream()), 'a3d_copy_channel')
    return dst


def conv2d_bwd_data(d, dz, w, dx, relu_mask=None):
    lib = _lib.load()
    ws, n = _ws().get(lib.a3d_conv2d_bwd_data_ws_bytes(ctypes.byref(d)), dz.device)
    check(lib.a3d_conv2d_bwd_data(ctypes.byref(d), _ptr(dz), _ptr(w), _ptr(dx), _ptr(relu_mask), ws, n, _stream()),
          'a3d_conv2d_bwd_data')
    return dx


def conv2d_bwd_filter(d, x, dz, dw, db=None):
    lib = _lib.load()
    ws, n = _ws().get(lib.a3d_conv2d_bwd_filter_ws_bytes(ctypes.byref(d)), x.device)
    check(lib.a3d_conv2d_bwd_filter(ctypes.byref(d), _ptr(x), _ptr(dz), _ptr(dw), _ptr(db), ws, n, _stream()),
          'a3d_conv2d_bwd_filter')
    return dw, db


def conv2d_bwd_filter_wino(d, x, dz, dw, db=None):
    lib = _lib.load()
    ws, n = _ws().get(lib.a3dwg_conv2d_bwd_filter_ws_bytes(ctypes.byref(d)), x.device)
    check(lib.a3dwg_conv2d_bwd_filter(ctypes.byref(d), _ptr(x), _ptr(dz), _ptr(dw), _ptr(db), ws, n, _stream()),
          'a3dwg_conv2d_bwd_filter')
    return dw, db


def conv2d_bwd_wino(d, x, dz, w, dw, db, dx, relu_mask=None, pool=None):
    lib = _lib.load()
    prepared = int(bool(d.hints & HINT_W_PREPARED))
    ws, n = _ws().get(lib.a3dwb_conv2d_bwd_ws_bytes(ctypes.byref(d), prepared, int(pool is not None)), x.device)
    pp = None
    if pool is not None:
        argmax, y = pool
        pp = ctypes.byref(_lib.WinoBwdPool(_ptr(argmax), _ptr(y), y.shape[-1], dx.shape[1], dx.shape[2]))
    check(lib.a3dwb_conv2d_bwd(ctypes.byref(d), _ptr(x), _ptr(dz), _ptr(w), _ptr(dw), _ptr(db), _ptr(dx), _ptr(relu_mask), pp,
                               ws, n, _stream()), 'a3dwb_conv2d_bwd')
    return dw, db, dx


def conv2d_bwd_filter_pooled_supported(d):
    return _lib.load().a3d_conv2d_bwd_filter_pooled_ws_bytes(ctypes.byref(d)) > 0


def conv2d_bwd_filter_pooled(d, x, dpool, pooled, argmax, dw, db=None):
    lib = _lib.load()
    ws, n = _ws().get(lib.a3d_conv2d_bwd_filter_pooled_ws_bytes(ctypes.byref(d)), x.device)
    assert pooled is None or (pooled.dtype == dpool.dtype and pooled.shape[-1] == dpool.shape[-1])
    check(lib.a3d_conv2d_bwd_filter_pooled(ctypes.byref(d), _ptr(x), _ptr(dpool), dpool.shape[-1], _ptr(pooled), _ptr(argmax),
                                           argmax.shape[-1], int(dpool.dtype == torch.bfloat16), _ptr(dw), _ptr(db), ws, n,
                                           _stream()), 'a3d_conv2d_bwd_filter_pooled')
    return dw, db


_BOTH_STATE = {}


def conv2d_bwd_both_supported(d):
    return bool(_lib.load().a3d_conv2d_bwd_both_supported(ctypes.byref(d)))


def conv2d_bwd_both(d, x, dz, w, dw, db, dx, relu_mask=True):
    lib = _lib.load()
    key = (torch.cuda.current_stream().cuda_stream, x.device)
    state = _BOTH_STATE.get(key)
    if state is None:
        state = _BOTH_STATE[key] = torch.zeros(64, dtype=torch.int32, device=x.device)
    ws, n = _ws().get(lib.a3d_conv2d_bwd_both_ws_bytes(ctypes.byref(d)), x.device)
    check(lib.a3d_conv2d_bwd_both(ctypes.byref(d), _ptr(x), _ptr(dz), _ptr(w), _ptr(dw), _ptr(db), _ptr(dx), dx.shape[-1],
                                  int(dx.dtype == torch.bfloat16), int(bool(relu_mask)), _ptr(state), ws, n, _stream()),
          'a3d_conv2d_bwd_both')
    return dw, db, dx


def dense_fwd(x, w, bias, y, act=None, drop_keep=None):
    m, k = x.shape
    n = w.shape[1]
    lib = _lib.load()
    ws, nb = _ws().get(lib.a3d_dense_fwd_ws_bytes(m, k, n), x.device)
    check(lib.a3d_dense_fwd(m, k, n, _ptr(x), _ptr(w), _ptr(bias), _ptr(y), ACT[act], _ptr(drop_keep), ws, nb,
                            _stream()), 'a3d_dense_fwd')
    return y


def dense_bwd_data(dz, w, dx, mask=None, scale=1.0, mask_act='relu'):
    m, n = dz.shape
    k = w.shape[0]
    lib = _lib.load()
    ws, nb = _ws().get(lib.a3d_dense_bwd_data_ws_bytes(m, k, n), dz.device)
    check(lib.a3d_dense_bwd_data(m, k, n, _ptr(dz), _ptr(w), _ptr(dx), _ptr(mask), ACT[mask_act], scale, ws, nb,
                                 _stream()),
          'a3d_dense_bwd_data')
    return dx


def dense_bwd_filter(x, dz, dw, db=None):
    m, k = x.shape
    n = dz.shape[1]
    lib = _lib.load()
    ws, nb = _ws().get(lib.a3d_dense_bwd_filter_ws_bytes(m, k, n), x.device)
    check(lib.a3d_dense_bwd_filter(m, k, n, _ptr(x), _ptr(dz), _ptr(dw), _ptr(db), ws, nb, _stream()),
          'a3d_dense_bwd_filter')
    return dw, db


def maxpool2x2_fwd(x, y, extra=None):
    n, h, w, c = x.shape
    check(_lib.load().a3d_maxpool2x2_fwd(n, h, w, c, _ptr(x), _ptr(y), y.shape[-1], _ptr(extra), _stream()),
          'a3d_maxpool2x2_fwd')
    return y


def maxpool2x2_bwd(x, dy, dx, relu_mask=True):
    n, h, w, c = x.shape
    check(_lib.load().a3d_maxpool2x2_bwd(n, h, w, c, _ptr(x), _ptr(dy), dy.shape[-1], _ptr(dx), int(relu_mask),
                                         _stream()), 'a3d_maxpool2x2_bwd')
    return dx


def _pair_args(x0, y0, x1=None, y1=None):
    def one(x, y):
        if x is None:
            return 0, None, 0, 0, 0, None
        return x.shape[3], _ptr(x), int(x.dtype == torch.uint8), y.shape[1], y.shape[2], _ptr(y)
    return tuple(x0.shape[:3]) + one(x0, y0) + one(x1, y1)


def resize_bilinear_tf1(x, y):
    n, h, w, c = x.shape
    if x.dtype == torch.uint8:
        check(_lib.load().a3d_resize_bilinear_tf1_ex(*_pair_args(x, y), _stream()), 'a3d_resize_bilinear_tf1_ex')
        return y
    check(_lib.load().a3d_resize_bilinear_tf1(n, h, w, c, _ptr(x), y.shape[1], y.shape[2], _ptr(y), _stream()),
          'a3d_resize_bilinear_tf1')
    return y


def resize_bilinear_tf1_pair(x0, y0, x1, y1):
    n, h, w, c0 = x0.shape
    assert x1.shape[:3] == (n, h, w)
    if x0.dtype == torch.uint8 or x1.dtype == torch.uint8:
        check(_lib.load().a3d_resize_bilinear_tf1_ex(*_pair_args(x0, y0, x1, y1), _stream()), 'a3d_resize_bilinear_tf1_ex')
        return
    check(_lib.load().a3d_resize_bilinear_tf1_pair(n, h, w, c0, _ptr(x0), y0.shape[1], y0.shape[2], _ptr(y0), x1.shape[3],
                                                   _ptr(x1), y1.shape[1], y1.shape[2], _ptr(y1), _stream()),
          'a3d_resize_bilinear_tf1_pair')


WARP_STRIDE = 12


def _check_pair(who, x0, y0, x1, y1, table):
    if x0.dim() != 4 or y0.dim() != 4 or y0.shape[0] != x0.shape[0] or y0.shape[3] != x0.shape[3]:
        raise ValueError(f'{who}: {tuple(x0.shape)} -> {tuple(y0.shape)}')
    n, h, w, c0 = x0.shape
    if (x1 is None) != (y1 is None):
        raise ValueError(f'{who}: x1 and y1 go together')
    if x1 is not None and (x1.dim() != 4 or tuple(x1.shape[:3]) != (n, h, w) or y1.dim() != 4
                           or y1.shape[0] != n or y1.shape[3] != x1.shape[3]):
        raise ValueError(f'{who}: second tensor {tuple(x1.shape)} -> {tuple(y1.shape)} beside '
                         f'{tuple(x0.shape)}')
    if table is not None and (tuple(table.shape) != (n, WARP_STRIDE) or table.dtype != torch.float32):
        raise ValueError(f'{who}: table {tuple(table.shape)} {table.dtype}, want [{n}, {WARP_STRIDE}] float32')
    for name, t, dtypes in (('x0', x0, (torch.float32, torch.uint8)), ('y0', y0, (torch.float32,)),
                            ('x1', x1, (torch.float32, torch.uint8)), ('y1', y1, (torch.float32,)),
                            ('table', table, (torch.float32,))):
        if t is None:
            continue
        if t.dtype not in dtypes:
            raise ValueError(f'{who}: {name} is {t.dtype}')
        if not t.is_cuda or t.device != x0.device:
            raise ValueError(f'{who}: {name} is on {t.device}, x0 on {x0.device}')
        if not t.is_contiguous():
            raise ValueError(f'{who}: {name} is not contiguous')
    return n, h, w, c0


# ... 934 lines not shown
```

Measured before the change: 12390.

## Add 1-D Winograd F(4,5) route for conv2d_1 backward data and filter

Adds a row-wise 1-D Winograd F(4,5) transform path for the backward data and backward filter passes of the coarse conv2d_1 layer. The input, dz and filter are transformed along the width axis, batched implicit GEMMs run over 8 transform planes, and the results are inverse-transformed, with the relu mask folded into the data-gradient output. This is meant to cut the multiply count of the wide-kernel convolution. In exchange it adds transform kernels, extra workspace traffic, and transform-matrix constants (entries up to 5.25) that may cost some fp32 accuracy. The fixup kernel body is also factored out into a reusable device function.

```diff
diff --git a/ann3depth_amd/_lib.py b/ann3depth_amd/_lib.py
--- a/ann3depth_amd/_lib.py
+++ b/ann3depth_amd/_lib.py
@@ -193,6 +193,15 @@
     'a3dwg_conv2d_bwd_filter': (c_int, [_D, _P, _P, _P, _P, _P, c_size_t, _P]),
 }
 
+WINO1D_SIGNATURES = {
+    'a3dl_conv2d_bwd_data_ws_bytes': (c_size_t, [_D]),
+    'a3dl_conv2d_bwd_data': (c_int, [_D, _P, _P, _P, _P, _P, c_size_t, _P]),
+    'a3dl_conv2d_bwd_filter_ws_bytes': (c_size_t, [_D]),
+    'a3dl_conv2d_bwd_filter': (c_int, [_D, _P, _P, _P, _P, _P, c_size_t, _P]),
+    'a3dl_conv2d_bwd_data_prepared_filter_bytes': (c_size_t, [_D]),
+    'a3dl_conv2d_bwd_data_prepare_filter': (c_int, [_D, _P, _P, c_size_t, _P]),
+}
+
 class WinoBwdPool(ctypes.Structure):
     _fields_ = [('argmax', c_void_p), ('y', c_void_p), ('ldy', c_int), ('h2', c_int), ('w2', c_int)]
 
@@ -242,6 +251,7 @@
     Surface('a3dh_', 'a3d_berhu.h', BERHU_SIGNATURES),
     Surface('a3da_', 'a3d_align.h', ALIGN_SIGNATURES),
     Surface('a3di_', 'a3d_ssi.h', SSI_SIGNATURES),
+    Surface('a3dl_', 'a3d_wino1d.h', WINO1D_SIGNATURES),
 )
 
 _lib = None
diff --git a/ann3depth_amd/csrc/a3d_internal.h b/ann3depth_amd/csrc/a3d_internal.h
--- a/ann3depth_amd/csrc/a3d_internal.h
+++ b/ann3depth_amd/csrc/a3d_internal.h
@@ -145,4 +145,34 @@
 int wino_bwd_finish(const a3d_conv_desc* d, const WinoGradGeom& gg, const float* slabs, const float* bparts, float* dw, float* db,
                     const float* M, float* dx, const float* mask, const WinoBwdPool* pool, hipStream_t st);
 
+struct Wino1dGeom {
+  int R, tw, off;
+  size_t Pv, Pm;
+  int K, N, Kp, Np;
+  int bn, tiles_m, tiles_n, nk, blocks;
+  size_t v_bytes, m_bytes, u_bytes;
+  size_t sk_bytes;
+};
+struct Wino1dGradGeom {
+  int R, tw;
+  size_t Px, Pz;
+  int Cp, Kp, splits;
+  size_t v_bytes, z_bytes;
+  size_t slab_bytes, bias_bytes;
+};
+int wino1d_bwd_blocks(long tiles, long nk);
+int wino1d_grad_splits(int M, int N, size_t pixels);
+Wino1dGeom wino1d_geom(const a3d_conv_desc* d);
+Wino1dGradGeom wino1d_grad_geom(const a3d_conv_desc* d);
+bool wino1d_applicable(const a3d_conv_desc* d);
+int wino1d_filter(const a3d_conv_desc* d, const float* w, float* U, hipStream_t st);
+int wino1d_input(const float* src, float* V, size_t rows, int W, int c, int ld, int off, int tw, int Cp, hipStream_t st);
+int wino1d_dz(const a3d_conv_desc* d, const Wino1dGradGeom& g, const float* dz, float* Z, hipStream_t st);
+int wino1d_output(const a3d_conv_desc* d, const Wino1dGeom& g, const float* M, float* dx, const float* mask, hipStream_t st);
+int wino1d_dw(const a3d_conv_desc* d, const Wino1dGradGeom& g, const float* slabs, const float* bparts, float* dw, float* db, hipStream_t st);
+a3d_timing_record wino1d_record(const Wino1dGeom& g);
+a3d_timing_record wino1d_grad_record(const a3d_conv_desc* d, const Wino1dGradGeom& g);
+int wino1d_gemm(IgemmParams& p, const Wino1dGeom& g, float* sk, hipStream_t st);
+int wino1d_grad_gemm(IgemmParams& p, const Wino1dGradGeom& g, hipStream_t st);
+
 }
diff --git a/ann3depth_amd/csrc/igemm.h b/ann3depth_amd/csrc/igemm.h
--- a/ann3depth_amd/csrc/igemm.h
+++ b/ann3depth_amd/csrc/igemm.h
@@ -1094,15 +1094,14 @@
 }
 
 template <int MODE, int BM, int BN, int WAVES_M, int NWAVES>
-__global__ __launch_bounds__(256) void igemm_fixup_kernel(const IgemmParams p, const uint32_t nblk) {
+__device__ __forceinline__ void igemm_fixup_body(const IgemmParams& p, const uint32_t nblk, const uint32_t tile, const uint32_t ygroup) {
   constexpr int WAVES_N = NWAVES / WAVES_M, WM = BM / WAVES_M, WN = BN / WAVES_N, TM = WM / 32, TN = WN / 32;
   constexpr int UNITS = NWAVES * TM * TN * 4;
   constexpr int MAXC = 1024;
   __shared__ uint32_t slots[MAXC];
   __shared__ uint32_t nslots;
   const int lane = threadIdx.x & 63;
-  const int unit = (int)blockIdx.y * 4 + (int)(threadIdx.x >> 6);
-  const uint32_t tile = blockIdx.x;
+  const int unit = (int)ygroup * 4 + (int)(threadIdx.x >> 6);
   const uint32_t nk = p.div_nk.d, tiles = (uint32_t)(p.tiles_m * p.tiles_n);
   if (threadIdx.x == 0) {
     uint32_t n = 0;
@@ -1147,12 +1146,16 @@
     store_quad<MODE>(p, s, tile_m * BM + wm * WM + a * 32 + 8 * q + 4 * lh, tile_n * BN + wn * WN + bb * 32 + li, p.C,
                      p.ldc, false);
   }
-  if (MODE == MODE_BWD_F && p.dbias != nullptr && tile_m == 0 && blockIdx.y == 0 && (int)threadIdx.x < BN) {
+  if (MODE == MODE_BWD_F && p.dbias != nullptr && tile_m == 0 && ygroup == 0 && (int)threadIdx.x < BN) {
     static_assert(BN <= 256, "bias sums by the first 256 threads");
     float bsum = 0.f;
     for (uint32_t i = 0; i < n; ++i) bsum += p.sk_bias[(size_t)slots[i] * BN + threadIdx.x];
     if (tile_n * BN + (int)threadIdx.x < p.N) p.dbias[tile_n * BN + threadIdx.x] = bsum;
   }
+}
+template <int MODE, int BM, int BN, int WAVES_M, int NWAVES>
+__global__ __launch_bounds__(256) void igemm_fixup_kernel(const IgemmParams p, const uint32_t nblk) {
+  igemm_fixup_body<MODE, BM, BN, WAVES_M, NWAVES>(p, nblk, blockIdx.x, blockIdx.y);
 }
 
 template <int MODE, int BM, int BN, int WAVES_M, int NWAVES, int BKT, int AVEC, int BVEC>
diff --git a/ann3depth_amd/csrc/igemm_host.hip b/ann3depth_amd/csrc/igemm_host.hip
--- a/ann3depth_amd/csrc/igemm_host.hip
+++ b/ann3depth_amd/csrc/igemm_host.hip
@@ -4,6 +4,7 @@
 #include "../../include/a3d_wino.h"
 #include "../../include/a3d_wino_grad.h"
 #include "../../include/a3d_wino_bwd.h"
+#include "../../include/a3d_wino1d.h"
 #include "a3d_internal.h"
 #include "igemm.h"
 #include "igemm_cfgs.h"
@@ -958,6 +959,118 @@
   return wino_bwd_finish(&e, gg, slabs, bparts, dw, db, M, dx, relu_mask, pool ? &wp : nullptr, st);
 }
 
+static bool wino1d_takes(const a3d_conv_desc* d) { return check_desc(d) == A3D_OK && wino1d_applicable(d); }
+
+static size_t wino1d_bytes(const Wino1dGeom& g, bool prepared) { return (prepared ? 0 : g.u_bytes) + g.v_bytes + g.m_bytes + g.sk_bytes; }
+static size_t wino1d_grad_bytes(const Wino1dGradGeom& g) { return g.v_bytes + g.z_bytes + g.slab_bytes + g.bias_bytes; }
+
+static IgemmParams wino1d_product(const a3d_conv_desc* d, const Wino1dGeom& g, const float* V, const float* U, float* M) {
+  a3d_conv_desc e{};
+  e.n = d->n; e.h = d->ho; e.w = g.tw; e.ho = d->h; e.wo = g.tw; e.c = g.Kp; e.k = g.Np; e.r = g.R; e.s = 1; e.stride = 1;
+  e.pad_t = g.R - 1 - d->pad_t; e.ldx = g.Kp; e.ldy = g.Np;
+  GemmProblem gp = fwd_problem(&e);
+  IgemmParams p;
+  fill_common(p, gp);
+  p.A = V; p.B = U; p.C = M;
+  p.npix = gp.M; p.nrsc = gp.K;
+  fill_gather(p, &e, g.Kp, 1, g.Kp);
+  p.ldb = g.Np; p.ldc = g.Np;
+  fill_staging(p, MODE_FWD, (unsigned long long)g.Pv * g.Kp, (unsigned long long)g.R * g.Kp * g.Np, g.R, 1);
+  return p;
+}
+static IgemmParams wino1d_grad_product(const a3d_conv_desc* d, const Wino1dGradGeom& g, const float* V, const float* Z, float* slabs,
+                                       float* bparts) {
+  a3d_conv_desc e{};
+  e.n = d->n; e.h = d->h; e.w = g.tw; e.ho = d->ho; e.wo = g.tw; e.c = g.Cp; e.k = g.Kp; e.r = g.R; e.s = 1; e.stride = 1;
+  e.pad_t = d->pad_t; e.ldx = g.Cp; e.ldy = g.Kp;
+  GemmProblem gp = bwd_f_problem(&e);
+  IgemmParams p;
+  fill_common(p, gp);
+  p.A = V; p.B = Z; p.C = slabs; p.dbias = bparts;
+  p.npix = gp.K; p.nrsc = gp.M;
+  fill_gather(p, &e, g.Cp, 1, g.Cp);
+  p.ldb = g.Kp; p.ldc = g.Kp;
+  fill_staging(p, MODE_BWD_F, (unsigned long long)g.Px * g.Cp, (unsigned long long)g.Pz * g.Kp, g.R, 1);
+  return p;
+}
+
+size_t a3dl_conv2d_bwd_data_ws_bytes(const a3d_conv_desc* d) {
+  if (!wino1d_takes(d)) return a3d_conv2d_bwd_data_ws_bytes(d);
+  return wino1d_bytes(wino1d_geom(d), (d->hints & A3D_HINT_W_PREPARED) != 0);
+}
+
+int a3dl_conv2d_bwd_data(const a3d_conv_desc* d, const float* dz, const float* w, float* dx, const float* relu_mask, void* ws,
+                         size_t ws_bytes, void* stream) {
+  if (!wino1d_takes(d)) return a3d_conv2d_bwd_data(d, dz, w, dx, relu_mask, ws, ws_bytes, stream);
+  A3D_CHECK_ARG(dz && w && dx, "conv2d_bwd_data (Winograd 1-D): null tensor");
+  A3D_CHECK_WS(ws, "conv2d_bwd_data (Winograd 1-D)");
+  const bool prepared = (d->hints & A3D_HINT_W_PREPARED) != 0;
+  const Wino1dGeom g = wino1d_geom(d);
+  const size_t need = wino1d_bytes(g, prepared);
+  if (!ws || need > ws_bytes) return set_error(A3D_EWORKSPACE, "conv2d_bwd_data (Winograd 1-D): need %zu workspace bytes", need);
+  A3D_CHECK_ARG(!prepared || aligned16(w), "conv2d_bwd_data (Winograd 1-D): the prepared filter must be 16-byte aligned");
+  hipStream_t st = static_cast<hipStream_t>(stream);
+  char* base = static_cast<char*>(ws);
+  const float* U = w;
+  int rc;
+  if (!prepared) {
+    rc = wino1d_filter(d, w, reinterpret_cast<float*>(base), st);
+    if (rc != A3D_OK) return rc;
+    U = reinterpret_cast<const float*>(base);
+    base += g.u_bytes;
+  }
+  float* V = reinterpret_cast<float*>(base);
+  float* M = reinterpret_cast<float*>(base + g.v_bytes);
+  float* sk = reinterpret_cast<float*>(base + g.v_bytes + g.m_bytes);
+  rc = wino1d_input(dz, V, (size_t)d->n * d->ho, d->wo, d->k, d->ldy, g.off, g.tw, g.Kp, st);
+  if (rc != A3D_OK) return rc;
+  IgemmParams p = wino1d_product(d, g, V, U, M);
+  rc = timed_launch(wino1d_record(g), st, [&] { return wino1d_gemm(p, g, sk, st); });
+  if (rc != A3D_OK) return rc;
+  return wino1d_output(d, g, M, dx, relu_mask, st);
+}
+
+size_t a3dl_conv2d_bwd_filter_ws_bytes(const a3d_conv_desc* d) {
+  if (!wino1d_takes(d)) return a3d_conv2d_bwd_filter_ws_bytes(d);
+  return wino1d_grad_bytes(wino1d_grad_geom(d));
+}
+
+int a3dl_conv2d_bwd_filter(const a3d_conv_desc* d, const float* x, const float* dz, float* dw, float* db, void* ws, size_t ws_bytes,
+                           void* stream) {
+  if (!wino1d_takes(d)) return a3d_conv2d_bwd_filter(d, x, dz, dw, db, ws, ws_bytes, stream);
+  A3D_CHECK_ARG(x && dz && dw, "conv2d_bwd_filter (Winograd 1-D): null tensor");
+  A3D_CHECK_WS(ws, "conv2d_bwd_filter (Winograd 1-D)");
+  const Wino1dGradGeom g = wino1d_grad_geom(d);
+  const size_t need = wino1d_grad_bytes(g);
+  if (!ws || need > ws_bytes) return set_error(A3D_EWORKSPACE, "conv2d_bwd_filter (Winograd 1-D): need %zu workspace bytes", need);
+  hipStream_t st = static_cast<hipStream_t>(stream);
+  char* base = static_cast<char*>(ws);
+  float* V = reinterpret_cast<float*>(base);
+  float* Z = reinterpret_cast<float*>(base + g.v_bytes);
+  float* slabs = reinterpret_cast<float*>(base + g.v_bytes + g.z_bytes);
+  float* bparts = reinterpret_cast<float*>(base + g.v_bytes + g.z_bytes + g.slab_bytes);
+  int rc = wino1d_input(x, V, (size_t)d->n * d->h, d->w, d->c, d->ldx, d->pad_l, g.tw, g.Cp, st);
+  if (rc != A3D_OK) return rc;
+  rc = wino1d_dz(d, g, dz, Z, st);
+  if (rc != A3D_OK) return rc;
+  IgemmParams p = wino1d_grad_product(d, g, V, Z, slabs, db ? bparts : nullptr);
+  rc = timed_launch(wino1d_grad_record(d, g), st, [&] { return wino1d_grad_gemm(p, g, st); });
+  if (rc != A3D_OK) return rc;
+  return wino1d_dw(d, g, slabs, bparts, dw, db, st);
+}
+
+size_t a3dl_conv2d_bwd_data_prepared_filter_bytes(const a3d_conv_desc* d) { return wino1d_takes(d) ? wino1d_geom(d).u_bytes : 0; }
+
+int a3dl_conv2d_bwd_data_prepare_filter(const a3d_conv_desc* d, const float* w, void* prepared, size_t prepared_bytes, void* stream) {
+  int rc = check_desc(d);
+  if (rc != A3D_OK) return rc;
+  A3D_CHECK_ARG(w && prepared && aligned16(prepared), "conv2d_bwd_data_prepare_filter (Winograd 1-D): null or misaligned buffer");
+  const size_t need = a3dl_conv2d_bwd_data_prepared_filter_bytes(d);
+  A3D_CHECK_ARG(need > 0, "conv2d_bwd_data_prepare_filter (Winograd 1-D): the route does not take this descriptor");
+  if (prepared_bytes < need) return set_error(A3D_EWORKSPACE, "conv2d_bwd_data_prepare_filter (Winograd 1-D): need %zu bytes", need);
+  return wino1d_filter(d, w, static_cast<float*>(prepared), static_cast<hipStream_t>(stream));
+}
+
 static a3d_conv_desc dense_desc(int m, int k, int n) {
   a3d_conv_desc d{};
   d.n = m; d.h = 1; d.w = 1; d.c = k; d.k = n; d.r = 1; d.s = 1; d.stride = 1; d.ho = 1; d.wo = 1;
diff --git a/ann3depth_amd/csrc/wino1d.hip b/ann3depth_amd/csrc/wino1d.hip
--- /dev/null
+++ b/ann3depth_amd/csrc/wino1d.hip
@@ -0,0 +1,382 @@
+#include "a3d_internal.h"
+#include "igemm.h"
+#include "igemm_cfgs.h"
+#include "wino1d_mats.h"
+
+namespace a3d {
+
+typedef float f4 __attribute__((ext_vector_type(4)));
+
+template <typename C, int ROWS, int COLS, const C (&Mx)[ROWS][COLS], bool TR, int J, int L, typename T>
+__device__ __forceinline__ void w1_dot(const T (&in)[TR ? ROWS : COLS], T& acc) {
+  if constexpr (L < (TR ? ROWS : COLS)) {
+    constexpr C c = TR ? Mx[L][J] : Mx[J][L];
+    if constexpr (c != C(0)) acc += c * in[L];
+    w1_dot<C, ROWS, COLS, Mx, TR, J, L + 1, T>(in, acc);
+  }
+}
+template <typename C, int ROWS, int COLS, const C (&Mx)[ROWS][COLS], bool TR, typename T, int J = 0>
+__device__ __forceinline__ void w1_apply(const T (&in)[TR ? ROWS : COLS], T (&out)[TR ? COLS : ROWS]) {
+  if constexpr (J < (TR ? COLS : ROWS)) {
+    T acc = T(0);
+    w1_dot<C, ROWS, COLS, Mx, TR, J, 0, T>(in, acc);
+    out[J] = acc;
+    w1_apply<C, ROWS, COLS, Mx, TR, T, J + 1>(in, out);
+  }
+}
+
+__global__ __launch_bounds__(256) void wino1d_filter_kernel(const float* __restrict__ w, float* __restrict__ U, int c, int k, int R, int Kp,
+                                                            int Np) {
+  const size_t plane = (size_t)R * Kp * Np;
+  for (size_t i = (size_t)blockIdx.x * 256 + threadIdx.x; i < plane; i += (size_t)gridDim.x * 256) {
+    const int col = (int)(i % Np), row = (int)((i / Np) % Kp), r = (int)(i / ((size_t)Np * Kp));
+    float g[5], u[8];
+#pragma unroll
+    for (int s = 0; s < 5; ++s) g[s] = (row < k && col < c) ? w[((size_t)((R - 1 - r) * 5 + (4 - s)) * c + col) * k + row] : 0.f;
+    w1_apply<float, 8, 5, kW1G, false, float>(g, u);
+#pragma unroll
+    for (int xi = 0; xi < 8; ++xi) U[(size_t)xi * plane + i] = u[xi];
+  }
+}
+
+template <bool VEC>
+__global__ __launch_bounds__(256) void wino1d_input_kernel(const float* __restrict__ src, float* __restrict__ V, int W, int c, int ld, int off,
+                                                           int tw, int Cp, size_t P) {
+  const int cqn = Cp / 4;
+  const size_t total = P * (size_t)cqn;
+  for (size_t i = (size_t)blockIdx.x * 256 + threadIdx.x; i < total; i += (size_t)gridDim.x * 256) {
+    const int cq = (int)(i % cqn);
+    const size_t pix = i / cqn, row = pix / tw;
+    const int x0 = 4 * (int)(pix % tw) - off;
+    f4 d[8], v[8];
+#pragma unroll
+    for (int b = 0; b < 8; ++b) {
+      f4 t = f4(0.f);
+      const int xx = x0 + b;
+      if (xx >= 0 && xx < W) {
+        const float* s = src + (row * W + xx) * (size_t)ld + cq * 4;
+        if (VEC) {
+          t = *reinterpret_cast<const f4*>(s);
+        } else {
+#pragma unroll
+          for (int e = 0; e < 4; ++e)
+            if (cq * 4 + e < c) t[e] = s[e];
+        }
+      }
+      d[b] = t;
+    }
+    w1_apply<float, 8, 8, kW1BT, false, f4>(d, v);
+#pragma unroll
+    for (int xi = 0; xi < 8; ++xi) *reinterpret_cast<f4*>(V + ((size_t)xi * P + pix) * Cp + cq * 4) = v[xi];
+  }
+}
+
+template <bool VEC>
+__global__ __launch_bounds__(256) void wino1d_dz_kernel(const float* __restrict__ dz, float* __restrict__ Z, int wo, int k, int ld, int tw, int Kp,
+                                                        size_t P) {
+  const int cqn = Kp / 4;
+  const size_t total = P * (size_t)cqn;
+  for (size_t i = (size_t)blockIdx.x * 256 + threadIdx.x; i < total; i += (size_t)gridDim.x * 256) {
+    const int cq = (int)(i % cqn);
+    const size_t pix = i / cqn, row = pix / tw;
+    const int x0 = 4 * (int)(pix % tw);
+    f4 y[4], z[8];
+#pragma unroll
+    for (int b = 0; b < 4; ++b) {
+      f4 t = f4(0.f);
+      if (x0 + b < wo) {
+        const float* s = dz + (row * wo + x0 + b) * (size_t)ld + cq * 4;
+        if (VEC) {
+          t = *reinterpret_cast<const f4*>(s);
+        } else {
+#pragma unroll
+          for (int e = 0; e < 4; ++e)
+            if (cq * 4 + e < k) t[e] = s[e];
+        }
+      }
+      y[b] = t;
+    }
+    w1_apply<float, 4, 8, kW1AT, true, f4>(y, z);
+#pragma unroll
+    for (int xi = 0; xi < 8; ++xi) *reinterpret_cast<f4*>(Z + ((size_t)xi * P + pix) * Kp + cq * 4) = z[xi];
+  }
+}
+
+template <bool VEC>
+__global__ __launch_bounds__(256) void wino1d_output_kernel(const float* __restrict__ M, float* __restrict__ out, const float* __restrict__ mask,
+                                                            int w, int ncols, int ld, int tw, int Np, size_t P) {
+  const int cqn = Np / 4;
+  const size_t total = P * (size_t)cqn;
+  for (size_t i = (size_t)blockIdx.x * 256 + threadIdx.x; i < total; i += (size_t)gridDim.x * 256) {
+    const int cq = (int)(i % cqn);
+    const size_t pix = i / cqn, row = pix / tw;
+    const int x0 = 4 * (int)(pix % tw);
+    f4 m[8], y[4];
+#pragma unroll
+    for (int xi = 0; xi < 8; ++xi) m[xi] = *reinterpret_cast<const f4*>(M + ((size_t)xi * P + pix) * Np + cq * 4);
+    w1_apply<float, 4, 8, kW1AT, false, f4>(m, y);
+#pragma unroll
+    for (int b = 0; b < 4; ++b) {
+      if (x0 + b >= w) continue;
+      const size_t o = (row * w + x0 + b) * (size_t)ld + cq * 4;
+      f4 v = y[b];
+      if (VEC) {
+        if (mask) {
+          const f4 a = *reinterpret_cast<const f4*>(mask + o);
+#pragma unroll
+          for (int e = 0; e < 4; ++e) v[e] = apply_act_grad(v[e], a[e], EPI_RELU, 1.f);
+        }
+        *reinterpret_cast<f4*>(out + o) = v;
+      } else {
+#pragma unroll
+        for (int e = 0; e < 4; ++e)
+          if (cq * 4 + e < ncols) out[o + e] = mask ? apply_act_grad(v[e], mask[o + e], EPI_RELU, 1.f) : v[e];
+      }
+    }
+  }
+}
+
+__global__ __launch_bounds__(256) void wino1d_dw_kernel(const float* __restrict__ slabs, const float* __restrict__ bparts, float* __restrict__ dw,
+                                                        float* __restrict__ db, int c, int k, int R, int Cp, int Kp, int splits) {
+  const size_t total = (size_t)R * c * k, plane = (size_t)R * Cp * Kp;
+  for (size_t i = (size_t)blockIdx.x * 256 + threadIdx.x; i < total; i += (size_t)gridDim.x * 256) {
+    const int col = (int)(i % k), row = (int)((i / k) % c), r = (int)(i / ((size_t)k * c));
+    const size_t at = ((size_t)r * Cp + row) * Kp + col;
+    double m[8], g[5];
+#pragma unroll
+    for (int xi = 0; xi < 8; ++xi) m[xi] = (double)slabs[(size_t)xi * splits * plane + at];
+    for (int z = 1; z < splits; ++z) {
+      float v[8];
+#pragma unroll
+      for (int xi = 0; xi < 8; ++xi) v[xi] = slabs[((size_t)xi * splits + z) * plane + at];
+#pragma unroll
+      for (int xi = 0; xi < 8; ++xi) m[xi] += (double)v[xi];
+    }
+    w1_apply<double, 8, 5, kW1Gd, true, double>(m, g);
+#pragma unroll
+    for (int s = 0; s < 5; ++s) dw[((size_t)(r * 5 + s) * c + row) * k + col] = (float)g[s];
+    if (db && r == 0 && row == 0) {
+      float s = bparts[col];
+      for (int z = 1; z < splits; ++z) s += bparts[(size_t)z * Kp + col];
+      db[col] = s;
+    }
+  }
+}
+
+struct Wino1dBatch {
+  size_t a, b, c, sk;
+};
+template <int BN, int WAVES_M, int NWAVES>
+__global__ __launch_bounds__(64 * NWAVES, 2 * NWAVES / 4) void wino1d_gemm_kernel(const IgemmParams p, const Wino1dBatch bt) {
+  IgemmParams q = p;
+  q.A = p.A + (size_t)blockIdx.y * bt.a;
+  q.B = p.B + (size_t)blockIdx.y * bt.b;
+  q.C = p.C + (size_t)blockIdx.y * bt.c;
+  q.sk_ws = p.sk_ws + (size_t)blockIdx.y * bt.sk;
+  igemm_body<MODE_FWD, 128, BN, WAVES_M, NWAVES, 32, 4, 4>(q, gridDim.x, blockIdx.x);
+}
+template <int BN, int WAVES_M, int NWAVES>
+__global__ __launch_bounds__(256) void wino1d_fixup_kernel(const IgemmParams p, const uint32_t nblk, const Wino1dBatch bt) {
+  IgemmParams q = p;
+  q.C = p.C + (size_t)blockIdx.z * bt.c;
+  q.sk_ws = p.sk_ws + (size_t)blockIdx.z * bt.sk;
+  igemm_fixup_body<MODE_FWD, 128, BN, WAVES_M, NWAVES>(q, nblk, blockIdx.x, blockIdx.y);
+}
+
+constexpr int kBM = 128, kBN = 128, kWavesM = 4, kNWaves = 8, kBK = 32;
+constexpr int kBiasPlane = 1;
+__global__ __launch_bounds__(64 * kNWaves, 2 * kNWaves / 4) void wino1d_grad_gemm_kernel(const IgemmParams p, const Wino1dBatch bt) {
+  IgemmParams q = p;
+  q.A = p.A + (size_t)blockIdx.y * bt.a;
+  q.B = p.B + (size_t)blockIdx.y * bt.b;
+  q.C = p.C + (size_t)blockIdx.y * bt.c;
+  if (blockIdx.y != kBiasPlane) q.dbias = nullptr;
+  igemm_body<MODE_BWD_F, kBM, kBN, kWavesM, kNWaves, kBK, 4, 4>(q, gridDim.x, blockIdx.x);
+}
+
+constexpr int kBlockSlots = 512, kCUs = 256, kPlanes = 8;
+
+constexpr int kMinShare = 4;
+int wino1d_bwd_blocks(long tiles, long nk) {
+  long b = std::max(1L, std::min((long)(kBlockSlots / kPlanes), tiles * nk / kMinShare));
+  const int forced = tune_int("A3D_WINO1D_BLOCKS", 0);
+  if (forced > 0) b = std::min((long)forced, std::min(tiles * nk, 128L));
+  return (int)b;
+}
+
+constexpr int kMinKTiles = 5;
+int wino1d_grad_splits(int M, int N, size_t pixels) {
+  const long blocks1 = (long)kPlanes * ((M + kBM - 1) / kBM) * ((N + kBN - 1) / kBN);
+  const long nk = (long)((pixels + kBK - 1) / kBK);
+  const long smax = std::max(1L, std::min(kBlockSlots / blocks1, nk / kMinKTiles));
+  long s = 1, load = (blocks1 + kCUs - 1) / kCUs;
+  for (long t = 2; t <= smax; ++t) {
+    const long l = (blocks1 * t + kCUs - 1) / kCUs;
+    if (l * s <= load * t) { s = t; load = l; }
+  }
+  const int forced = tune_int("A3D_WINO1D_GRAD_SPLIT", 0);
+  if (forced > 0) s = std::min((long)forced, nk);
+  const long per = (nk + s - 1) / s;
+  return (int)((nk + per - 1) / per);
+}
+
+static size_t up256(size_t b) { return (b + 255) / 256 * 256; }
+
+Wino1dGeom wino1d_geom(const a3d_conv_desc* d) {
+  Wino1dGeom g{};
+  g.R = d->r;
+  g.tw = (d->w + 3) / 4;
+  g.off = 4 - d->pad_l;
+  g.Pv = (size_t)d->n * d->ho * g.tw;
+  g.Pm = (size_t)d->n * d->h * g.tw;
+  g.K = d->k; g.N = d->c;
+  g.Kp = (g.K + 3) / 4 * 4;
+  g.Np = (g.N + 3) / 4 * 4;
+  g.bn = g.Np <= 96 ? 96 : 128;
+  g.tiles_m = (int)((g.Pm + 127) / 128);
+  g.tiles_n = (g.Np + g.bn - 1) / g.bn;
+  g.nk = (g.R * g.Kp + kBK - 1) / kBK;
+  g.blocks = wino1d_bwd_blocks((long)g.tiles_m * g.tiles_n, g.nk);
+  g.v_bytes = up256((size_t)kPlanes * g.Pv * g.Kp * 4);
+  g.m_bytes = up256((size_t)kPlanes * g.Pm * g.Np * 4);
+  g.u_bytes = up256((size_t)kPlanes * g.R * g.Kp * g.Np * 4);
+  g.sk_bytes = up256((size_t)kPlanes * 2 * g.blocks * 128 * g.bn * 4);
+  return g;
+}
+
+Wino1dGradGeom wino1d_grad_geom(const a3d_conv_desc* d) {
+  Wino1dGradGeom g{};
+  g.R = d->r;
+  g.tw = (d->wo + 3) / 4;
+  g.Px = (size_t)d->n * d->h * g.tw;
+  g.Pz = (size_t)d->n * d->ho * g.tw;
+  g.Cp = (d->c + 3) / 4 * 4;
+  g.Kp = (d->k + 3) / 4 * 4;
+  g.splits = wino1d_grad_splits(g.R * g.Cp, g.Kp, g.Pz);
+  g.v_bytes = up256((size_t)kPlanes * g.Px * g.Cp * 4);
+  g.z_bytes = up256((size_t)kPlanes * g.Pz * g.Kp * 4);
+  g.slab_bytes = up256((size_t)kPlanes * g.splits * g.R * g.Cp * g.Kp * 4);
+  g.bias_bytes = up256((size_t)g.splits * g.Kp * 4);
+  return g;
+}
+
+bool wino1d_applicable(const a3d_conv_desc* d) {
+  if (d->precision != A3D_PREC_F32 || d->storage || d->s != 5 || d->stride != 1 || d->pad_l > 4) return false;
+  const Wino1dGeom g = wino1d_geom(d);
+  const Wino1dGradGeom gg = wino1d_grad_geom(d);
+  const double lim = 2147483647.0;
+  for (double bytes : {(double)g.Pv * g.Kp, (double)g.Pm * g.Np, (double)g.R * g.Kp * g.Np, (double)gg.Px * gg.Cp, (double)gg.Pz * gg.Kp,
+                       (double)g.R * gg.Cp * gg.Kp})
+    if (bytes * 4.0 >= lim) return false;
+  return true;
+}
+
+int wino1d_filter(const a3d_conv_desc* d, const float* w, float* U, hipStream_t st) {
+  const Wino1dGeom g = wino1d_geom(d);
+  clear_stale_error();
+  hipLaunchKernelGGL(wino1d_filter_kernel, dim3(grid_for((size_t)g.R * g.Kp * g.Np)), dim3(256), 0, st, w, U, d->c, d->k, g.R, g.Kp, g.Np);
+  return check_launch("wino1d_filter");
+}
+
+int wino1d_input(const float* src, float* V, size_t rows, int W, int c, int ld, int off, int tw, int Cp, hipStream_t st) {
+  const size_t P = rows * tw;
+  const bool vec = c % 4 == 0 && ld % 4 == 0 && aligned16(src);
+  const dim3 grid(grid_for(P * (size_t)(Cp / 4), 256, 1u << 20)), block(256);
+  clear_stale_error();
+  if (vec) hipLaunchKernelGGL(wino1d_input_kernel<true>, grid, block, 0, st, src, V, W, c, ld, off, tw, Cp, P);
+  else hipLaunchKernelGGL(wino1d_input_kernel<false>, grid, block, 0, st, src, V, W, c, ld, off, tw, Cp, P);
+  return check_launch("wino1d_input");
+}
+
+int wino1d_dz(const a3d_conv_desc* d, const Wino1dGradGeom& g, const float* dz, float* Z, hipStream_t st) {
+  const bool vec = d->k % 4 == 0 && d->ldy % 4 == 0 && aligned16(dz);
+  const dim3 grid(grid_for(g.Pz * (size_t)(g.Kp / 4), 256, 1u << 20)), block(256);
+  clear_stale_error();
+  if (vec) hipLaunchKernelGGL(wino1d_dz_kernel<true>, grid, block, 0, st, dz, Z, d->wo, d->k, d->ldy, g.tw, g.Kp, g.Pz);
+  else hipLaunchKernelGGL(wino1d_dz_kernel<false>, grid, block, 0, st, dz, Z, d->wo, d->k, d->ldy, g.tw, g.Kp, g.Pz);
+  return check_launch("wino1d_dz");
+}
+
+int wino1d_output(const a3d_conv_desc* d, const Wino1dGeom& g, const float* M, float* dx, const float* mask, hipStream_t st) {
+  const bool vec = g.N % 4 == 0 && d->ldx % 4 == 0 && aligned16(dx) && aligned16(mask);
+  const dim3 grid(grid_for(g.Pm * (size_t)(g.Np / 4), 256, 1u << 20)), block(256);
+  clear_stale_error();
+  if (vec) hipLaunchKernelGGL(wino1d_output_kernel<true>, grid, block, 0, st, M, dx, mask, d->w, g.N, d->ldx, g.tw, g.Np, g.Pm);
+  else hipLaunchKernelGGL(wino1d_output_kernel<false>, grid, block, 0, st, M, dx, mask, d->w, g.N, d->ldx, g.tw, g.Np, g.Pm);
+  return check_launch("wino1d_output");
+}
+
+int wino1d_dw(const a3d_conv_desc* d, const Wino1dGradGeom& g, const float* slabs, const float* bparts, float* dw, float* db, hipStream_t st) {
+  clear_stale_error();
+  hipLaunchKernelGGL(wino1d_dw_kernel, dim3(grid_for((size_t)g.R * d->c * d->k, 256, 1u << 20)), dim3(256), 0, st, slabs, bparts, dw, db, d->c,
+                     d->k, g.R, g.Cp, g.Kp, g.splits);
+  return check_launch("wino1d_dw");
+}
+
+a3d_timing_record wino1d_record(const Wino1dGeom& g) {
+  return timing_record(MODE_BWD_D, A3D_PREC_F32, 128, g.bn, 4, g.bn == 96 ? 4 : 8, kBK, 4, 4, 0, (int)(kPlanes * g.Pm), g.N, g.R * g.K);
+}
+a3d_timing_record wino1d_grad_record(const a3d_conv_desc* d, const Wino1dGradGeom& g) {
+  a3d_timing_record r = timing_record(MODE_BWD_F, A3D_PREC_F32, kBM, kBN, kWavesM, kNWaves, kBK, 4, 4, 0, g.R * d->c, d->k, (int)(kPlanes * g.Pz));
+  r.splitk = g.splits;
+  return r;
+}
+
+static int raise_lds(const void* kern, size_t bytes, bool (&done)[64]) {
+  int dev = 0;
+  (void)hipGetDevice(&dev);
+  if (dev < 0 || dev >= 64 || !done[dev]) {
+    hipError_t e = hipFuncSetAttribute(kern, hipFuncAttributeMaxDynamicSharedMemorySize, (int)bytes);
+    if (e != hipSuccess) return set_error(A3D_ELAUNCH, "hipFuncSetAttribute: %s", hipGetErrorString(e));
+    if (dev >= 0 && dev < 64) done[dev] = true;
+  }
+  return A3D_OK;
+}
+
+template <int BN, int WAVES_M, int NWAVES>
+static int wino1d_gemm_as(IgemmParams& p, const Wino1dGeom& g, const Wino1dBatch& bt, hipStream_t st) {
+  using Cfg = IgemmCfg<MODE_FWD, 128, BN, WAVES_M, NWAVES, 32, 4, 4>;
+  static bool attr_done[64] = {};
+  int rc = raise_lds(reinterpret_cast<const void*>(wino1d_gemm_kernel<BN, WAVES_M, NWAVES>), Cfg::LDS_BYTES, attr_done);
+  if (rc != A3D_OK) return rc;
+  clear_stale_error();
+  hipLaunchKernelGGL((wino1d_gemm_kernel<BN, WAVES_M, NWAVES>), dim3((unsigned)g.blocks, kPlanes), dim3(Cfg::NT), Cfg::LDS_BYTES, st, p, bt);
+  rc = check_launch("wino1d_gemm");
+  if (rc != A3D_OK) return rc;
+  hipLaunchKernelGGL((wino1d_fixup_kernel<BN, WAVES_M, NWAVES>), dim3((unsigned)(g.tiles_m * g.tiles_n), (128 * BN / 256 + 3) / 4, kPlanes),
+                     dim3(256), 0, st, p, (uint32_t)g.blocks, bt);
+  return check_launch("wino1d_fixup");
+}
+
+int wino1d_gemm(IgemmParams& p, const Wino1dGeom& g, float* sk, hipStream_t st) {
+  p.splitk = 1;
+  p.ktiles_per_split = g.nk;
+  p.tiles_m = g.tiles_m;
+  p.tiles_n = g.tiles_n;
+  p.slab = (size_t)p.M * p.N;
+  p.streamk = 1;
+  p.sk_ws = sk;
+  p.div_nk = make_fastdiv((uint32_t)g.nk);
+  const Wino1dBatch bt{g.Pv * (size_t)g.Kp, (size_t)g.R * g.Kp * g.Np, g.Pm * (size_t)g.Np, (size_t)2 * g.blocks * 128 * g.bn};
+  if (g.bn == 96) return wino1d_gemm_as<96, 4, 4>(p, g, bt, st);
+  return wino1d_gemm_as<128, 4, 8>(p, g, bt, st);
+}
+
+int wino1d_grad_gemm(IgemmParams& p, const Wino1dGradGeom& g, hipStream_t st) {
+  using Cfg = IgemmCfg<MODE_BWD_F, kBM, kBN, kWavesM, kNWaves, kBK, 4, 4>;
+  static bool attr_done[64] = {};
+  const int rc = raise_lds(reinterpret_cast<const void*>(wino1d_grad_gemm_kernel), Cfg::LDS_BYTES, attr_done);
+  if (rc != A3D_OK) return rc;
+  const int nk = (p.K + kBK - 1) / kBK;
+  p.splitk = g.splits;
+  p.ktiles_per_split = (nk + g.splits - 1) / g.splits;
+  p.tiles_m = (p.M + kBM - 1) / kBM;
+  p.tiles_n = (p.N + kBN - 1) / kBN;
+  p.slab = (size_t)p.M * p.N;
+  const Wino1dBatch bt{g.Px * (size_t)g.Cp, g.Pz * (size_t)g.Kp, (size_t)g.splits * p.slab, 0};
+  clear_stale_error();
+  hipLaunchKernelGGL(wino1d_grad_gemm_kernel, dim3((unsigned)(p.tiles_m * p.tiles_n * p.splitk), kPlanes), dim3(Cfg::NT), Cfg::LDS_BYTES, st, p, bt);
+  return check_launch("wino1d_grad_gemm");
+}
+
+}
diff --git a/ann3depth_amd/csrc/wino1d_mats.h b/ann3depth_amd/csrc/wino1d_mats.h
--- /dev/null
+++ b/ann3depth_amd/csrc/wino1d_mats.h
@@ -0,0 +1,49 @@
+#pragma once
+
+namespace a3d {
+
+constexpr float kW1G[8][5] = {
+    {-1.0f, 0.0f, 0.0f, 0.0f, 0.0f},
+    {-0.2222222238779068f, -0.2222222238779068f, -0.2222222238779068f, -0.2222222238779068f, -0.2222222238779068f},
+    {-0.2222222238779068f, 0.2222222238779068f, -0.2222222238779068f, 0.2222222238779068f, -0.2222222238779068f},
+    {0.011111111380159855f, 0.02222222276031971f, 0.04444444552063942f, 0.08888889104127884f, 0.17777778208255768f},
+    {0.011111111380159855f, -0.02222222276031971f, 0.04444444552063942f, -0.08888889104127884f, 0.17777778208255768f},
+    {0.7111111283302307f, 0.35555556416511536f, 0.17777778208255768f, 0.08888889104127884f, 0.04444444552063942f},
+    {0.7111111283302307f, -0.35555556416511536f, 0.17777778208255768f, -0.08888889104127884f, 0.04444444552063942f},
+    {0.0f, 0.0f, 0.0f, 0.0f, 1.0f},
+};
+constexpr double kW1Gd[8][5] = {
+    {-1.0, 0.0, 0.0, 0.0, 0.0},
+    {-0.2222222222222222, -0.2222222222222222, -0.2222222222222222, -0.2222222222222222, -0.2222222222222222},
+    {-0.2222222222222222, 0.2222222222222222, -0.2222222222222222, 0.2222222222222222, -0.2222222222222222},
+    {0.011111111111111112, 0.022222222222222223, 0.044444444444444446, 0.08888888888888889, 0.17777777777777778},
+    {0.011111111111111112, -0.022222222222222223, 0.044444444444444446, -0.08888888888888889, 0.17777777777777778},
+    {0.7111111111111111, 0.35555555555555557, 0.17777777777777778, 0.08888888888888889, 0.044444444444444446},
+    {0.7111111111111111, -0.35555555555555557, 0.17777777777777778, -0.08888888888888889, 0.044444444444444446},
+    {0.0, 0.0, 0.0, 0.0, 1.0},
+};
+constexpr bool w1_g_tables_agree() {
+  for (int j = 0; j < 8; ++j)
+    for (int k = 0; k < 5; ++k)
+      if ((float)kW1Gd[j][k] != kW1G[j][k]) return false;
+  return true;
+}
+static_assert(w1_g_tables_agree(), "kW1G is kW1Gd rounded to float");
+constexpr float kW1AT[4][8] = {
+    {1.0f, 1.0f, 1.0f, 1.0f, 1.0f, 1.0f, 1.0f, 0.0f},
+    {0.0f, 1.0f, -1.0f, 2.0f, -2.0f, 0.5f, -0.5f, 0.0f},
+    {0.0f, 1.0f, 1.0f, 4.0f, 4.0f, 0.25f, 0.25f, 0.0f},
+    {0.0f, 1.0f, -1.0f, 8.0f, -8.0f, 0.125f, -0.125f, 1.0f},
+};
+constexpr float kW1BT[8][8] = {
+    {-1.0f, 0.0f, 5.25f, 0.0f, -5.25f, 0.0f, 1.0f, 0.0f},
+    {0.0f, 1.0f, 1.0f, -4.25f, -4.25f, 1.0f, 1.0f, 0.0f},
+    {0.0f, -1.0f, 1.0f, 4.25f, -4.25f, -1.0f, 1.0f, 0.0f},
+    {0.0f, 0.5f, 0.25f, -2.5f, -1.25f, 2.0f, 1.0f, 0.0f},
+    {0.0f, -0.5f, 0.25f, 2.5f, -1.25f, -2.0f, 1.0f, 0.0f},
+    {0.0f, 2.0f, 4.0f, -2.5f, -5.0f, 0.5f, 1.0f, 0.0f},
+    {0.0f, -2.0f, 4.0f, 2.5f, -5.0f, -0.5f, 1.0f, 0.0f},
+    {0.0f, -1.0f, 0.0f, 5.25f, 0.0f, -5.25f, 0.0f, 1.0f},
+};
+
+}
diff --git a/ann3depth_amd/models.py b/ann3depth_amd/models.py
--- a/ann3depth_amd/models.py
+++ b/ann3depth_amd/models.py
@@ -310,6 +310,15 @@
                 d = self.d[n]
                 if d.n * -(-d.ho // 2) * -(-d.wo // 2) >= self.WINO_GRAD_MIN_TILES:
                     self.wino_grad.add(n)
+        self.wino1d_bwd_d, self.wino1d_bwd_f = set(), set()
+        if precision == 'fp32' and dev.type == 'cuda':
+            for n in self.WINO1D_LAYERS:
+                d = self.d[n]
+                rows = d.n * d.h * -(-d.w // 4)
+                if rows >= self.WINO1D_BWD_D_MIN_ROWS:
+                    self.wino1d_bwd_d.add(n)
+                if rows >= self.WINO1D_BWD_F_MIN_ROWS:
+                    self.wino1d_bwd_f.add(n)
         self.d_few = {}
         if dev.type == 'cuda':
             few_prec = 'bf16' if self.bf16s else 'fp32'
@@ -355,6 +364,10 @@
     WINO_GRAD_MIN_TILES = 504
     WINO_BWD_CHAIN = True
 
+    WINO1D_LAYERS = ('coarse/conv/conv2d_1',)
+    WINO1D_BWD_D_MIN_ROWS = 2160
+    WINO1D_BWD_F_MIN_ROWS = 2160
+
     def _desc(self, name, which):
         d = self.d[name]
         bits = self.store.get(name, {}).get(which, 0)
@@ -776,6 +789,10 @@
         d, w = self._desc(name, 'bwd_d'), self._w(name, 'bwd_d')
         if name in self.d_wino:
             d, w = self._prepared((name, 'bwd_d', 'fp32w'), self.d_wino[name], w, 'bwd_d')
+        if name in self.wino1d_bwd_d:
+            d, w = self._prepared((name, 'bwd_d', 'wino1d'), d, w, 'bwd_d_wino1d')
+            ops.conv2d_bwd_data_wino1d(d, dz, w, dx, relu_mask=relu_mask)
+            return
         ops.conv2d_bwd_data(d, dz, w, dx, relu_mask=relu_mask)
 
     def _wino_chain(self, name):
@@ -788,6 +805,8 @@
     def _bwd_filter(self, name, x, dz):
         if name in self.d:
             call = ops.conv2d_bwd_filter_wino if name in self.wino_grad else ops.conv2d_bwd_filter
+            if name in self.wino1d_bwd_f:
+                call = ops.conv2d_bwd_filter_wino1d
             call(self._desc(name, 'bwd_f'), x, dz, self._g(name + '/kernel'), self._g(name + '/bias'))
         elif self._fused_dense_adam():
             g = self.groups[self.group_of[name + '/kernel']]
diff --git a/ann3depth_amd/ops.py b/ann3depth_amd/ops.py
--- a/ann3depth_amd/ops.py
+++ b/ann3depth_amd/ops.py
@@ -67,7 +67,7 @@
 
     def __init__(self, desc, device, which='fwd'):
         lib = _lib.load()
-        self.stem = {'fwd': 'a3d_conv2d_fwd', 'bwd_d': 'a3dw_conv2d_bwd_data'}[which]
+        self.stem = {'fwd': 'a3d_conv2d_fwd', 'bwd_d': 'a3dw_conv2d_bwd_data', 'bwd_d_wino1d': 'a3dl_conv2d_bwd_data'}[which]
         nbytes = getattr(lib, self.stem + '_prepared_filter_bytes')(ctypes.byref(desc))
         self.ok = nbytes > 0
         self.desc = desc
@@ -172,6 +172,22 @@
     ws, n = _ws().get(lib.a3dwg_conv2d_bwd_filter_ws_bytes(ctypes.byref(d)), x.device)
     check(lib.a3dwg_conv2d_bwd_filter(ctypes.byref(d), _ptr(x), _ptr(dz), _ptr(dw), _ptr(db), ws, n, _stream()),
           'a3dwg_conv2d_bwd_filter')
+    return dw, db
+
+
+def conv2d_bwd_data_wino1d(d, dz, w, dx, relu_mask=None):
+    lib = _lib.load()
+    ws, n = _ws().get(lib.a3dl_conv2d_bwd_data_ws_bytes(ctypes.byref(d)), dz.device)
+    check(lib.a3dl_conv2d_bwd_data(ctypes.byref(d), _ptr(dz), _ptr(w), _ptr(dx), _ptr(relu_mask), ws, n, _stream()),
+          'a3dl_conv2d_bwd_data')
+    return dx
+
+
+def conv2d_bwd_filter_wino1d(d, x, dz, dw, db=None):
+    lib = _lib.load()
+    ws, n = _ws().get(lib.a3dl_conv2d_bwd_filter_ws_bytes(ctypes.byref(d)), x.device)
+    check(lib.a3dl_conv2d_bwd_filter(ctypes.byref(d), _ptr(x), _ptr(dz), _ptr(dw), _ptr(db), ws, n, _stream()),
+          'a3dl_conv2d_bwd_filter')
     return dw, db
 
 
diff --git a/include/a3d_wino1d.h b/include/a3d_wino1d.h
--- /dev/null
+++ b/include/a3d_wino1d.h
@@ -0,0 +1,24 @@
+#ifndef A3D_WINO1D_H_
+#define A3D_WINO1D_H_
+
+#include "a3d.h"
+
+#ifdef __cplusplus
+extern "C" {
+#endif
+
+size_t a3dl_conv2d_bwd_data_ws_bytes(const a3d_conv_desc* d);
+int a3dl_conv2d_bwd_data(const a3d_conv_desc* d, const float* dz, const float* w, float* dx, const float* relu_mask, void* ws,
+                         size_t ws_bytes, void* stream);
+
+size_t a3dl_conv2d_bwd_filter_ws_bytes(const a3d_conv_desc* d);
+int a3dl_conv2d_bwd_filter(const a3d_conv_desc* d, const float* x, const float* dz, float* dw, float* db, void* ws, size_t ws_bytes,
+                           void* stream);
+
+size_t a3dl_conv2d_bwd_data_prepared_filter_bytes(const a3d_conv_desc* d);
+int a3dl_conv2d_bwd_data_prepare_filter(const a3d_conv_desc* d, const float* w, void* prepared, size_t prepared_bytes, void* stream);
+
+#ifdef __cplusplus
+}
+#endif
+#endif
```

New measurement: 13800, median of 6. 1.11x the previous value.
